# will-rowe/groot

Measured on AMD Instinct MI355X. Metric: Mreads/s aligned, higher is better.
Workload: dtype u64

## Files before the change

groot_amd/csrc/hip/align.hip:

```cpp
#include <hip/hip_runtime.h>

#include "kernels_align.hpp"
#include "kernels_lean.hpp"
#include "launch.hpp"

namespace groot {

void launch_align(uint32_t pw, const AlignArgs &a, dim3 grid, hipStream_t st)
{
    const size_t lds = a.lds_stride_dw ? (size_t)kBlock * a.lds_stride_dw * 4 + 16 : 0;
    if (pw == 3) {
        if (lds) hipLaunchKernelGGL((align_kernel<3, true>), grid, dim3(kBlock), lds, st, a);
        else hipLaunchKernelGGL((align_kernel<3, false>), grid, dim3(kBlock), 0, st, a);
    } else if (pw == 11) {
        if (lds) hipLaunchKernelGGL((align_kernel<11, true>), grid, dim3(kBlock), lds, st, a);
        else hipLaunchKernelGGL((align_kernel<11, false>), grid, dim3(kBlock), 0, st, a);
    }
}

void launch_align_lean(uint32_t pw, const LeanArgs &a, dim3 grid, hipStream_t st)
{
    if (pw != 3) return;
    const size_t lds = (size_t)kBlock * a.lds_stride_dw * 4;
    if (a.max_len <= 128) hipLaunchKernelGGL((align_lean_kernel<3, 4>), grid, dim3(kBlock), lds, st, a);
    else if (a.max_len <= 160) hipLaunchKernelGGL((align_lean_kernel<3, 5>), grid, dim3(kBlock), lds, st, a);
    else hipLaunchKernelGGL((align_lean_kernel<3, 8>), grid, dim3(kBlock), lds, st, a);
}

}
```

groot_amd/csrc/hip/device_types.hpp:

```cpp
#pragma once

#include <cstdint>

#include <hip/hip_runtime.h>

#include "groot_hip.h"

namespace groot {

constexpr int kBlock = 256;
constexpr uint32_t kEmpty = 0xFFFFFFFFu;

enum : uint32_t {
    kFlagShortRead = 1u,
    kFlagLongRead = 2u,
    kFlagSeedOverflow = 4u,
    kFlagTravOverflow = 8u,
    kFlagOrdOverflow = 16u,
    kFlagOvfOverflow = 32u,
    kFlagQOverflow = 64u,
};

constexpr uint32_t kIncrCap = 8;
constexpr uint32_t kIncrCapBig = 2048;
constexpr uint32_t kSeedShards = 64, kSeedShardStride = 16;
constexpr uint32_t kOvfShards = 256;

struct DeviceCounters {
    unsigned long long mapped, multimapped, alignments, seeds, revcomp_panics, short_reads;
    unsigned int n_trav;
    unsigned int max_seeds;
    unsigned int flags;
    unsigned int q_rows;
    unsigned int mask_words;
    unsigned int todo_reads;
    unsigned int seeded_reads;
    unsigned int tab_reads;
    unsigned int lean_reads;
    unsigned long long dbg[192];
};

template <int PW> struct alignas(16) NodeRec {
    uint32_t seq_off;
    uint32_t seq_len;
    uint32_t deg;
    uint8_t child_first[4];
    uint64_t first8;
    uint32_t edges[4];
    uint64_t mask[PW];
};
static_assert(sizeof(NodeRec<3>) == 64, "node record must be one 64-byte line");
static_assert(sizeof(NodeRec<11>) == 128, "wide node record must be 128 bytes");

struct alignas(16) WinRec {
    uint32_t graph;
    uint32_t node;
    uint32_t offset;
    uint32_t l1_hi;
    uint32_t cn_off, cn_end;
    uint32_t seed_s0, seed_len;
};
static_assert(sizeof(WinRec) == 32, "window record is two 16-byte words");

struct alignas(16) ReadRec {
    uint64_t seq_off;
    uint32_t len;
    uint32_t cnt_flags;
    uint32_t seed[4];
};
static_assert(sizeof(ReadRec) == 32, "read record is two 16-byte words");

constexpr uint32_t kRecCountMask = 0x00FFFFFFu;
constexpr uint32_t kRecNo12F = 1u << 24, kRecNo3F = 1u << 25, kRecNo4F = 1u << 26;
constexpr uint32_t kRecPacked = 1u << 31;
constexpr uint32_t kRecAscending = 1u << 30;
constexpr uint32_t kLongListCap = 1u << 20, kSortSeedsMax = 512;
constexpr uint32_t kSplitMin = 8, kSplitMaxItems = 256;
constexpr uint32_t kRecSplit = 1u << 23;
constexpr uint32_t kPrefixWords = 256;

struct groot_ctrav {
    uint32_t node, offset;
    uint32_t read_flags;
};
static_assert(sizeof(groot_ctrav) == 12, "packed traversal record is 12 bytes");

constexpr uint32_t kOutHdrDw = 6, kOutSeedDw = 4;
constexpr uint32_t kOutTab = 0x80000000u;
constexpr uint32_t kOutMaxTrav = 4095, kOutIdxBits = 25, kOutTravShift = 27, kOutTravLong = 15;
constexpr uint32_t kOutNoRec = 1u << 25;
constexpr uint32_t kOutAllSeeds = 1u << 26;
constexpr uint32_t kTabSeedsHere = 0x40000000u;
constexpr uint32_t kTabCounted = 0x80000000u;
__host__ __device__ inline uint32_t out_stride_q(uint32_t pw)
{
    uint32_t q = 4;
    while (q * 16 < (kOutHdrDw + kOutSeedDw) * 4 + 8 * pw) q <<= 1;
    return q;
}

__host__ __device__ constexpr uint32_t text_key_dwords(uint32_t dw) { return dw <= 7 ? 7u : dw <= 8 ? 8u : 14u; }
__host__ __device__ constexpr uint32_t text_exc_dwords(uint32_t tw)
{
    return tw > 14 ? 0u : ((2 + tw) % 4 ? 4 - (2 + tw) % 4 : (tw <= 10 ? 4u : 0u));
}

struct ExactEntry { uint32_t tag; uint32_t id; };

struct alignas(32) SigEntry {
    uint32_t id;
    uint32_t cls;
    uint32_t text_len;
    uint32_t group;
    uint8_t verdict[2][8];
};
static_assert(sizeof(SigEntry) == 32, "signature entry is two 16-byte words");
constexpr uint32_t kSigInline = 1u << 30;
constexpr uint32_t kTextMax = 256;
__host__ __device__ inline uint32_t sig_text_pack(uint32_t len, uint32_t argmin_fwd, uint32_t argmin_rc) { return len | (argmin_fwd << 10) | (argmin_rc << 20); }
__host__ __device__ inline uint32_t sig_text_len(uint32_t v) { return v & 1023u; }
__host__ __device__ inline uint32_t sig_text_argmin(uint32_t v, uint32_t row) { return (v >> (10 + 10 * row)) & 1023u; }
// ... 70 lines not shown
struct AlignArgs {
    DeviceIndex ix;
    const uint8_t *seq;
    const uint64_t *seq_off;
    uint32_t n_reads, first_read_id;
    uint32_t seed_slots;
    const uint32_t *seed_count;
    const uint32_t *seed_win;
    const uint32_t *perm;
    const ReadRec *read_rec;
    uint32_t no_align, update_weights;
    const void *node_rec;
    uint32_t *attempts;
    groot_trav *trav_first;
    uint64_t *mask_first;
    uint32_t *trav_cnt;
    groot_trav *ovf_trav;
    uint64_t *ovf_mask;
    uint32_t *ovf_cnt;
    uint32_t ovf_cap;
    uint64_t *stk_hdr;
    uint64_t *stk_mask;
    uint32_t n_threads, stk_depth;
    uint32_t lds_stride_dw;
    uint32_t *incr_cnt, *incr_win;
    uint32_t incr_cap;
    uint32_t head_lanes;
    uint32_t round_lanes;
    const uint4 *vitem;
    const uint32_t *vcount;
    uint32_t vcap;
    const uint32_t *n_perm;
    uint32_t refill;
    DeviceCounters *ctr;
};

struct alignas(16) LeanNode {
    uint32_t seq_off;
    uint32_t seq_len;
    uint32_t deg_kids;
    uint32_t pad;
    uint32_t edges[4];
    uint64_t first32;
    uint64_t mask[3];
};
static_assert(sizeof(LeanNode) == 64, "lean node record is one 64-byte line");
constexpr uint32_t kLeanNo = 0x80000000u;
struct alignas(16) LeanExt {
    uint64_t b[7];
    uint64_t pad;
};
static_assert(sizeof(LeanExt) == 64, "lean node extension is one 64-byte line");
constexpr uint32_t kLeanMaxLen = 256;

struct LeanArgs {
    const LeanNode *nodes;
    const LeanExt *ext;
    const uint32_t *bases2;
    const uint4 *cn_pre2;
    const uint64_t *node_l2b;
    const uint8_t *win_ok;
    const WinRec *win_rec;
    const uint32_t *q_row;
    const uint8_t *seq;
    const uint4 *packed;
    uint32_t packed_q;
    const uint32_t *perm;
    const ReadRec *read_rec;
    uint32_t n_reads, first_read_id, n_windows, k;
    uint32_t update_weights;
    uint32_t lds_stride_dw;
    uint32_t max_len;
    uint32_t *attempts;
    groot_trav *trav_first;
    uint64_t *mask_first;
    uint32_t *trav_cnt;
    uint8_t *defer;
    uint4 *stk;
    groot_trav *ovf_trav;
    uint64_t *ovf_mask;
    uint32_t *ovf_cnt;
    uint32_t ovf_cap;
    DeviceCounters *ctr;
};

__host__ __device__ inline uint32_t lean_stride_dw(uint32_t max_len) { return (((max_len + 15u) >> 4) + 15u) | 1u; }

}
```

groot_amd/csrc/hip/groot_hip.hip:

```cpp
#include <cstring>

#include <hip/hip_runtime.h>
#include <rocprim/rocprim.hpp>

#include <dlfcn.h>

#include <algorithm>
#include <cmath>
#include <cstdarg>
#include <cstdio>
#include <atomic>
#include <chrono>
#include <deque>
#include <memory>
#include <numeric>
#include <string>
#include <thread>
#include <vector>

#include "../common/cpus.hpp"
#include "../common/view_check.hpp"
#include "kernels_misc.hpp"
#include "launch.hpp"

using namespace groot;

template <class T> struct DevBuf {
    T *p = nullptr;
    size_t n = 0;
    hipError_t alloc(size_t count)
    {
        release();
        n = count;
        return hipMalloc((void **)&p, std::max<size_t>(count, 1) * sizeof(T));
    }
    hipError_t reserve(size_t count) { return count <= n && p ? hipSuccess : alloc(count); }
    void release()
    {
        if (p) (void)hipFree(p);
        p = nullptr;
        n = 0;
    }
    ~DevBuf() { release(); }
};

template <class T> struct PinBuf {
    T *p = nullptr;
    size_t n = 0;
    hipError_t alloc(size_t count)
    {
        release();
        n = count;
        return hipHostMalloc((void **)&p, std::max<size_t>(count, 1) * sizeof(T), hipHostMallocDefault);
    }
    hipError_t reserve(size_t count) { return count <= n && p ? hipSuccess : alloc(count); }
    void release()
    {
        if (p) (void)hipHostFree(p);
        p = nullptr;
        n = 0;
    }
    ~PinBuf() { release(); }
};

struct Knobs {
    bool no_outcome_table = false, no_text_table = false, no_sig = false, force_rccl = false, small_buffers = false, open_stats = false, poison = false, lean = false;
    static Knobs read()
    {
        Knobs k;
        k.no_outcome_table = getenv("GROOT_NO_OUTCOME_TABLE") != nullptr; k.no_text_table = getenv("GROOT_NO_TEXT_TABLE") != nullptr;
        k.no_sig = getenv("GROOT_NO_SIG") != nullptr;                     k.force_rccl = getenv("GROOT_FORCE_RCCL") != nullptr;
        k.small_buffers = getenv("GROOT_TEST_SMALL_BUFFERS") != nullptr;  k.open_stats = getenv("GROOT_OPEN_STATS") != nullptr;
        k.poison = getenv("GROOT_TEST_POISON") != nullptr;
        k.lean = getenv("GROOT_LEAN") != nullptr;
        return k;
    }
};

struct Slot {
    enum State { FREE, ACQUIRED, IN_FLIGHT, D2H_ISSUED, COLLECTED };
    State state = FREE;
    uint64_t ticket = 0;
    uint32_t n_reads = 0, first_read_id = 0, max_len = 0;
    uint32_t set = 0;
    uint32_t uniform_len = 0;
    bool mixed_len = false;
    bool text_used = false;
    bool sig_used = false;
    uint32_t packed_q = 0;
    bool lean_used = false;
    bool one_len = false;
    uint64_t n_bases = 0, n_exc = 0;
    enum Input { IN_ASCII, IN_PACKED, IN_PACKED16, IN_DEVICE } input = IN_ASCII;
    const uint8_t *ext_seq = nullptr;
    const uint64_t *ext_off = nullptr;
    PinBuf<uint8_t> h_bases;
    PinBuf<uint16_t> h_len;
    PinBuf<uint64_t> h_off, h_exc_pos;
    PinBuf<uint8_t> h_exc_byte;
    DevBuf<uint16_t> d_len;
    DevBuf<uint32_t> d_packed;
    bool exc_at_home = false;
    DevBuf<uint8_t> d_seq, d_exc_byte;
    DevBuf<uint64_t> d_off, d_exc_pos;
    uint32_t trav_cap = 0;
    DevBuf<groot_trav> d_trav;
    DevBuf<uint64_t> d_mask;
    DevBuf<DeviceCounters> d_ctr;
    PinBuf<DeviceCounters> h_ctr;
    PinBuf<groot_trav> h_trav;
    DevBuf<groot_ctrav> d_ctrav;
    PinBuf<groot_ctrav> h_ctrav;
    PinBuf<uint8_t> h_mask;
    PinBuf<uint32_t> h_ckpt;
    DevBuf<uint8_t> d_cmask;
    DevBuf<uint32_t> d_mwords, d_moff, d_ckpt;
    uint32_t n_trav = 0, copied = 0;
    uint64_t n_mask_bytes = 0, copied_bytes = 0;
    bool host_results = false;
    hipEvent_t ev_seed = nullptr;
    hipEvent_t ev_h2d0 = nullptr, ev_h2d = nullptr, ev_compute = nullptr, ev_ctr = nullptr, ev_d2h0 = nullptr, ev_d2h = nullptr;
    hipEvent_t ev[14]{};
    groot_counts counts{};
    int status = GROOT_OK;
    std::string status_msg;
    groot_stage_ms ms{};
    const uint8_t *seq() const { return input == IN_DEVICE ? ext_seq : d_seq.p; }
    const uint64_t *off() const { return input == IN_DEVICE ? ext_off : d_off.p; }
};

struct WorkSet {
    DevBuf<uint32_t> seed_count, seed_win, perm, perm_count, trav_cnt, tab_idx;
    DevBuf<uint32_t> perm2, perm2_count;
    DevBuf<uint8_t> defer;
    DevBuf<uint4> packed;
    DevBuf<ReadRec> read_rec;
    DevBuf<uint4> vitem, split_list;
    DevBuf<uint32_t> vcount;
    DevBuf<groot_trav> trav_first;
    DevBuf<uint64_t> mask_first, sketches;
    hipEvent_t ev_free = nullptr;
    bool used = false;
    Slot *owner = nullptr;
    uint64_t ticket = 0;
};

struct groot_ctx {
    int device = 0;
    std::string err;
    groot_params prm{};
    Knobs kn;
    uint32_t s = 0, k = 0, max_k = 0, l_max = 0, pw_view = 0, pw = 0, n_windows = 0, max_q = 0, band_hash_bits = 0;
    hipEvent_t h2d_last = nullptr;
    Slot *newest = nullptr;
    hipEvent_t last_compute = nullptr;
    hipStream_t own_stream = nullptr, stream = nullptr, astream = nullptr, h2d_stream = nullptr, d2h_stream = nullptr;
    bool profiling = false;

    DevBuf<uint32_t> graph_win_end;
    DevBuf<uint4> cn_pre;
    DevBuf<uint64_t> node_l2b;
    DevBuf<uint32_t> win_prefix, edges, win_graph, cn_node,
        band_keys, band_ids;
    DevBuf<ExactEntry> band_hash;
    DevBuf<uint8_t> band_sig;
    DevBuf<uint32_t> band_run;
    DevBuf<uint8_t> bases, q_k, q_l;
    DevBuf<uint16_t> q_min_eq;
    DevBuf<uint64_t> win_sketch;
    DevBuf<unsigned char> node_rec;
    DevBuf<LeanExt> lean_ext;
    DevBuf<LeanNode> lean_nodes;
    DevBuf<uint32_t> bases2;
    DevBuf<uint4> cn_pre2;
    DevBuf<uint8_t> win_ok;
    DevBuf<uint4> lean_stk;
    bool lean = false;
    DevBuf<WinRec> win_rec;
    DevBuf<ExactEntry> exact;
    DevBuf<SigEntry> sig;
    DevBuf<uint4> sig_dir;
    DevBuf<uint8_t> win_text, win_nodes;
    DevBuf<uint32_t> sig_info;
    DevBuf<uint4> out_tab;
    std::vector<uint32_t> h_out_tab;
    uint64_t out_strings = 0, out_tabulated = 0, out_entries = 0;
    double out_build_ms = 0, open_ms = 0;
    uint32_t incr_cap = kIncrCap;
    bool tab_capture = false;
    DevBuf<uint32_t> tab_idx, tab_hist, incr_cnt, incr_win;
    DevBuf<uint4> text_tab;
    uint64_t text_entries = 0;
    uint32_t batches_without_text = 0, text_retry_gap = 8;
    double text_hit_frac = 1.0;
    std::vector<uint16_t> h_q_min_eq;
    uint32_t sig_disabled = 0;
    DeviceIndex dix{};

    std::thread bg;
    std::atomic<int> bg_state{0};
    std::atomic<bool> bg_cancel{false};
    int bg_rc = 0;
    std::string bg_err;
    DeviceIndex bg_dix{};
    uint32_t bg_seed_slots = 0, bg_max_read_len = 0;
    hipStream_t bg_stream = nullptr;
    DevBuf<unsigned long long> bg_shards;
    DeviceIndex *build_dix = nullptr;
    hipStream_t build_stream = nullptr;
    unsigned long long *build_shards = nullptr;

    std::vector<std::unique_ptr<Slot>> slots;
    std::deque<Slot *> inflight;
    uint64_t next_ticket = 1;
    Slot *waited = nullptr;
    double todo_frac = 1.0;
    double lean_left_frac = 1.0;
    uint32_t n_cu = 256;
    double dfs_frac = 1.0;
    double trav_per_read = 1.25;
    double bytes_per_trav = 0;
    bool packed_travs = false;
    std::vector<uint32_t> h_node_graph;
    DevBuf<uint8_t> graph_words;
    std::vector<uint8_t> h_graph_words;
    WorkSet ws[2];
    uint32_t next_set = 0;

    uint32_t seed_slots = 0;
    DevBuf<uint32_t> sort_key, sort_key_out, perm_in, todo_list, todo_count;
    DevBuf<uint32_t> long_list, long_count;
    uint32_t vcap = 0;
    uint32_t lsh_defer_rows = 0, lsh_cap = 0;
    DevBuf<unsigned long long> seed_shards;
    DevBuf<uint32_t> lsh_list, lsh_count;
    DevBuf<uint64_t> lsh_sketch;
    DevBuf<char> sort_tmp, in_tmp;
    uint32_t ovf_cap = 0;
    DevBuf<groot_trav> ovf_trav;
    DevBuf<uint64_t> ovf_mask;
    DevBuf<uint32_t> trav_off, ovf_cnt;
    DevBuf<char> scan_tmp;
    uint32_t align_threads = 0, stk_depth = 0;
    DevBuf<uint64_t> stk_hdr, stk_mask;
    DevBuf<uint32_t> attempts, q_row, q_seen, q_of_row, q_nrows;
    uint32_t *attempts_ptr = nullptr;
    uint32_t att_cap = 0;
    bool att_external = false;
};

__attribute__((constructor)) static void groot_hw_queues() { setenv("GPU_MAX_HW_QUEUES", "8", 0); }

static thread_local std::string g_open_err;

static thread_local bool tl_background = false;

static int fail(groot_ctx *ctx, int code, const char *fmt, ...)
{
    char buf[1024];
    va_list ap;
    va_start(ap, fmt);
    vsnprintf(buf, sizeof buf, fmt, ap);
    va_end(ap);
    if (ctx) (tl_background ? ctx->bg_err : ctx->err) = buf;
    else g_open_err = buf;
    return code;
}

#define HIP_TRY(ctx, expr)                                                                             \
    do {                                                                                                \
        hipError_t e__ = (expr);                                                                        \
        if (e__ != hipSuccess) return fail(ctx, GROOT_E_DEVICE, "%s: %s", #expr, hipGetErrorString(e__)); \
    } while (0)

template <class T> static hipError_t upload(DevBuf<T> &d, const T *src, size_t n, size_t pad = 0)
{
    hipError_t e = d.alloc(n + pad);
    if (e != hipSuccess) return e;
    if (pad) {
        e = hipMemset(d.p, 0, (n + pad) * sizeof(T));
        if (e != hipSuccess) return e;
    }
    if (n) e = hipMemcpy(d.p, src, n * sizeof(T), hipMemcpyHostToDevice);
    return e;
}

namespace {

struct KLProb {
    int x, q, l, k;
    double p(double t) const { return 1.0 - std::pow(1.0 - std::pow(t / (1.0 + double(x) / double(q) - t), double(k)), double(l)); }
};

template <class F> double integrate(F f, double a, double b, double precision)
{
    double area = 0.0;
    for (double x = a; x < b; x += precision) area += f(x + 0.5 * precision) * precision;
    return area;
}

void optimal_kl(int max_k, int max_l, int x, int q, double t, int &opt_k, int &opt_l)
{
    const double prec = 0.01;
    double min_err = 1.7976931348623157e308;
    opt_k = 0; opt_l = 0;
    const double xq = double(x) / double(q);
    for (int l = 1; l <= max_l; l++)
        for (int k = 1; k <= max_k; k++) {
            KLProb pr{x, q, l, k};
            double fp = 0.0, fn = 0.0;
            if (xq >= 1.0) {
                fp = integrate([&](double v) { return pr.p(v); }, 0.0, t, prec);
                fn = integrate([&](double v) { return 1.0 - pr.p(v); }, t, 1.0, prec);
            } else if (xq >= t) {
                fp = integrate([&](double v) { return pr.p(v); }, 0.0, t, prec);
                fn = integrate([&](double v) { return 1.0 - pr.p(v); }, t, xq, prec);
            }
            const double err = fn + fp;
            if (min_err > err) { min_err = err; opt_k = k; opt_l = l; }
        }
}

uint32_t min_equal_slots(uint32_t s, int q_size, int x_size, double t)
{
    if (q_size == 0 || x_size == 0) return s + 1;
    for (uint32_t eq = 1; eq <= s; eq++) {
        const double jaccard = double(eq) / double(s);
        const double c = (double(x_size) / double(q_size) + 1.0) * jaccard / (1.0 + jaccard);
        if (c > t) return eq;
    }
    return s + 1;
}

uint32_t round_pw(uint32_t pw)
{
    for (uint32_t c : {3u, 11u})
        if (pw <= c) return c;
    return 0;
}

template <int PW> void build_node_records(const groot_index_view *v, std::vector<unsigned char> &out)
{
    std::vector<NodeRec<PW>> recs(v->n_nodes);
    for (uint32_t n = 0; n < v->n_nodes; n++) {
        NodeRec<PW> &r = recs[n];
        memset(&r, 0, sizeof r);
        r.seq_off = v->node_seq_off[n];
        r.seq_len = v->node_seq_off[n + 1] - v->node_seq_off[n];
        const uint32_t e0 = v->node_edge_off[n], deg = v->node_edge_off[n + 1] - e0;
        bool wild = false;
        for (uint32_t i = 0; i < r.seq_len; i++) wild |= v->bases[r.seq_off + i] == 'N';
        r.deg = deg | (wild ? 0x80000000u : 0u);
        if (deg <= 4) {
            for (uint32_t e = 0; e < deg; e++) {
                const uint32_t c = v->edges[e0 + e];
                r.edges[e] = c;
                r.child_first[e] = v->node_seq_off[c] < v->node_seq_off[c + 1] ? v->bases[v->node_seq_off[c]] : (uint8_t)0;
            }
        } else {
            r.edges[0] = e0;
        }
        for (uint32_t i = 0; i < 8 && i < r.seq_len; i++) r.first8 |= (uint64_t)v->bases[r.seq_off + i] << (8 * i);
        for (uint32_t w = 0; w < v->path_words; w++) r.mask[w] = v->node_mask[(size_t)n * v->path_words + w];
    }
    out.resize(recs.size() * sizeof(NodeRec<PW>));
    if (!recs.empty()) memcpy(out.data(), recs.data(), out.size());
}

}

static constexpr uint32_t kMaxLdsReadBytes = 64 * 1024;

static int alloc_seed_slots(groot_ctx *c, uint32_t slots)
{
    c->seed_slots = slots;
    for (WorkSet &w : c->ws) { HIP_TRY(c, w.seed_win.alloc((size_t)slots * c->prm.max_batch_reads)); w.owner = nullptr; w.ticket = 0; }
    return GROOT_OK;
}

static int alloc_trav(groot_ctx *c, Slot *s, uint32_t cap)
{
    s->trav_cap = cap;
    HIP_TRY(c, s->d_trav.alloc((size_t)cap + 2));
    HIP_TRY(c, s->d_mask.alloc((size_t)cap * c->pw_view + 2));
    if (!c->prm.results_on_device) {
        HIP_TRY(c, s->h_trav.alloc((size_t)cap + 2));
        HIP_TRY(c, s->h_mask.alloc((size_t)cap * c->pw_view * 8 + 16));
        HIP_TRY(c, s->h_ckpt.alloc((size_t)cap / 256 + 2));
        HIP_TRY(c, s->d_cmask.alloc((size_t)cap * c->pw_view * 8 + 16));
        HIP_TRY(c, s->d_mwords.alloc(cap));
        HIP_TRY(c, s->d_moff.alloc(cap));
        HIP_TRY(c, s->d_ckpt.alloc((size_t)cap / 256 + 2));
        if (c->packed_travs) {
            HIP_TRY(c, s->d_ctrav.alloc((size_t)cap + 2));
            HIP_TRY(c, s->h_ctrav.alloc((size_t)cap + 2));
        }
    }
    return GROOT_OK;
}

static int alloc_ovf(groot_ctx *c, uint32_t cap_per_shard)
{
    c->ovf_cap = cap_per_shard;
    HIP_TRY(c, c->ovf_trav.alloc((size_t)kOvfShards * cap_per_shard));
    HIP_TRY(c, c->ovf_mask.alloc((size_t)kOvfShards * cap_per_shard * c->pw));
    return GROOT_OK;
}

static int grow_attempts(groot_ctx *c, uint32_t rows)
{
    if (c->att_external) return fail(c, GROOT_E_NOSPACE, "a kmerCount outside the fixed layout of groot_hip_attempts_layout occurred");
    DevBuf<uint32_t> bigger;
    HIP_TRY(c, bigger.alloc((size_t)rows * c->n_windows));
    HIP_TRY(c, hipMemset(bigger.p, 0, (size_t)rows * c->n_windows * sizeof(uint32_t)));
    if (c->attempts.p && c->att_cap)
        HIP_TRY(c, hipMemcpy(bigger.p, c->attempts.p, (size_t)std::min(rows, c->att_cap) * c->n_windows * sizeof(uint32_t), hipMemcpyDeviceToDevice));
    std::swap(c->attempts.p, bigger.p);
    std::swap(c->attempts.n, bigger.n);
    c->attempts_ptr = c->attempts.p;
    c->att_cap = rows;
    return GROOT_OK;
// ... 15 lines not shown
#define GROOT_HEAVY_BLOCKS 16384u
#endif
#ifndef GROOT_SORTLIST_BLOCKS
#define GROOT_SORTLIST_BLOCKS 16384
#endif
static int launch_seed_stage(groot_ctx *c, Slot *s, bool update_weights)
{
    WorkSet *w = &c->ws[s->set];
    SeedArgs a{};
    s->packed_q = 0;
    a.ix = c->dix;
    a.seq = s->seq();
    a.seq_off = s->off();
    a.n_reads = s->n_reads;
    a.max_read_len = c->prm.max_read_len;
    const uint64_t want = (uint64_t)kBlock * s->max_len + 32;
    a.lds_read_bytes = (uint32_t)std::min<uint64_t>(want, kMaxLdsReadBytes);
    a.seed_slots = c->seed_slots;
    a.seed_count = w->seed_count.p;
    a.seed_win = w->seed_win.p;
    a.sketch_out = c->prm.keep_sketches ? w->sketches.p : nullptr;
    a.sort_key = c->sort_key.p;
    a.read_rec = w->read_rec.p;
    a.q_seen = c->q_seen.p;
    a.trav_cnt = w->trav_cnt.p;
    a.shards = c->seed_shards.p;
    a.ctr = s->d_ctr.p;
    a.long_list = c->long_list.p; a.long_count = c->long_count.p;
    if (c->dix.out_tab) {
        a.tab_idx = w->tab_idx.p;
        a.tab_hist = c->tab_hist.p;
    }
    unsigned win_bits = 2;
    for (uint32_t v = c->n_windows ? c->n_windows - 1 : 0; v; v >>= 1) win_bits++;
    win_bits = std::min(32u, std::max(3u, win_bits));
    a.sort_span_bits = std::min((unsigned)GROOT_SPAN_BITS, 32u - win_bits);
    if (win_bits - 2u + a.sort_span_bits > 24u && win_bits - 2u + 4u <= 24u) a.sort_span_bits = 24u - (win_bits - 2u);
    a.sort_span_shift = win_bits;
    const unsigned begin_bit = 2u, end_bit = win_bits + a.sort_span_bits;
    const dim3 grid((s->n_reads + kBlock - 1) / kBlock);
#ifndef GROOT_LIST_BLOCKS_MIN
#define GROOT_LIST_BLOCKS_MIN 1280
#endif
    const uint32_t list_blocks = std::max<uint32_t>(GROOT_LIST_BLOCKS_MIN, (uint32_t)std::min<double>(4.0e6, c->todo_frac * 1.25 * (double)s->n_reads / kBlock + 1.0));
    bool sig_useful = true;
    if (s->one_len && s->max_len >= c->k) {
        const uint32_t q = s->max_len - c->k + 1;
        sig_useful = q < c->h_q_min_eq.size() && c->h_q_min_eq[q] == c->s;
    }
    s->sig_used = c->dix.sig && !c->prm.keep_sketches && sig_useful;
    const double list_below = kSparseBelow;
    const bool list_mode = c->dfs_frac < list_below;
    const bool text_try = c->text_hit_frac >= 0.7 || ++c->batches_without_text >= c->text_retry_gap;
    s->text_used = !c->prm.keep_sketches && c->dix.text_tab && c->dix.out_tab && text_try && s->max_len >= c->dix.w && !c->tab_capture;
    if (s->text_used) c->batches_without_text = 0;
    if (c->lsh_list.p && !c->prm.keep_sketches) {
        a.lsh_list = c->lsh_list.p; a.lsh_count = c->lsh_count.p; a.lsh_sketch = c->lsh_sketch.p;
        a.lsh_defer_rows = c->lsh_defer_rows; a.lsh_cap = c->lsh_cap;
        HIP_TRY(c, hipMemsetAsync(c->lsh_count.p, 0, 2 * sizeof(uint32_t), c->stream));
    }
    HIP_TRY(c, hipMemsetAsync(w->vcount.p, 0, 2 * sizeof(uint32_t), c->stream));
    if (c->profiling) HIP_TRY(c, hipEventRecord(s->ev[7], c->stream));
    if (s->text_used) {
        a.todo_list = c->todo_list.p;
        a.todo_count = c->todo_count.p;
        const uint32_t stride_dw = ((s->max_len + 3) / 4 + 1) | 1u;
        a.list_stride_dw = list_lds_stride(stride_dw);
        const size_t lds = kTextBad + (size_t)((a.lds_read_bytes + 15) / 16) * 4 + 96;
        HIP_TRY(c, hipMemsetAsync(c->todo_count.p, 0, sizeof(uint32_t), c->stream));
        if (list_mode) {
            a.dfs_list = w->perm.p; a.dfs_count = w->perm_count.p;
            HIP_TRY(c, hipMemsetAsync(w->perm_count.p, 0, sizeof(uint32_t), c->stream));
        }
        launch_text_lookup(text_key_dwords((c->dix.w + 15) / 16), a, grid, lds, c->stream);
        HIP_TRY(c, hipGetLastError());
        if (c->profiling) HIP_TRY(c, hipEventRecord(s->ev[8], c->stream));
        launch_list(c->s, a, dim3(std::min<uint32_t>(grid.x, list_blocks)), c->stream);
    } else if (s->sig_used) {
        a.todo_list = c->todo_list.p;
        a.todo_count = c->todo_count.p;
        const uint32_t stride_dw = ((s->max_len + 3) / 4 + 1) | 1u;
        a.list_stride_dw = list_lds_stride(stride_dw);
        HIP_TRY(c, hipMemsetAsync(c->todo_count.p, 0, sizeof(uint32_t), c->stream));
        if (c->lean && !c->tab_capture && w->packed.p) { a.packed = w->packed.p; a.packed_q = s->max_len <= 128 ? 2u : 4u; }
        s->packed_q = a.packed ? a.packed_q : 0;
        launch_sig(c->s, a, s->max_len, c->stream);
        HIP_TRY(c, hipGetLastError());
        if (c->profiling) HIP_TRY(c, hipEventRecord(s->ev[8], c->stream));
        launch_list(c->s, a, dim3(std::min<uint32_t>(grid.x, list_blocks)), c->stream);
    } else {
        const size_t lds = kLdsReads + ((a.lds_read_bytes + 15) & ~15u);
        launch_seed(c->s, c->max_k, a, c->prm.keep_sketches != 0, grid, lds, c->stream);
        HIP_TRY(c, hipGetLastError());
        if (c->profiling) HIP_TRY(c, hipEventRecord(s->ev[8], c->stream));
    }
    if (a.lsh_list) hipLaunchKernelGGL(lsh_heavy_kernel, dim3(std::min<uint32_t>(grid.x, GROOT_HEAVY_BLOCKS)), dim3(kBlock), 0, c->stream, a);
    HIP_TRY(c, hipGetLastError());
    if (c->profiling) HIP_TRY(c, hipEventRecord(s->ev[12], c->stream));
    {
        SplitArgs sa{};
        sa.list = c->long_list.p; sa.count = c->long_count.p; sa.seed_count = w->seed_count.p; sa.seed_win = w->seed_win.p;
        sa.n_reads = s->n_reads; sa.seed_slots = c->seed_slots; sa.read_rec = w->read_rec.p; sa.win_rec = c->dix.win_rec;
        sa.split = c->vcap && !c->tab_capture && !c->prm.no_exact_align;
        sa.vitem = w->vitem.p; sa.vcount = w->vcount.p; sa.vcap = c->vcap; sa.split_list = w->split_list.p;
        sa.ctr = s->d_ctr.p; sa.update_weights = update_weights ? 1 : 0;
        hipLaunchKernelGGL(sort_seed_lists_kernel, dim3(GROOT_SORTLIST_BLOCKS), dim3(kBlock), 0, c->stream, sa);
    }
    if (c->profiling) HIP_TRY(c, hipEventRecord(s->ev[2], c->stream));
    hipLaunchKernelGGL(assign_q_rows_kernel, dim3(1), dim3(64), 0, c->stream, c->q_seen.p, c->q_row.p, c->q_of_row.p, c->q_nrows.p, c->att_cap,
                       c->max_q, s->d_ctr.p, c->seed_shards.p, c->long_count.p);
    if (a.tab_hist) {
        hipLaunchKernelGGL(fold_tab_hist_kernel, dim3(std::min<uint32_t>((c->n_windows + kBlock - 1) / kBlock, 1024u)), dim3(kBlock), 0, c->stream, c->tab_hist.p,
                           c->attempts_ptr, c->q_row.p, c->dix.w - c->k + 1, c->n_windows, s->d_ctr.p, update_weights ? 1u : 0u);
        HIP_TRY(c, hipGetLastError());
    }
    if (list_mode && a.dfs_list) return GROOT_OK;
    if (list_mode) {
        size_t tb = 0;
        HasKey pred{c->sort_key.p};
        rocprim::counting_iterator<uint32_t> ids(0u);
        HIP_TRY(c, rocprim::select(nullptr, tb, ids, w->perm.p, w->perm_count.p, (size_t)s->n_reads, pred, c->stream));
        if (tb > c->sort_tmp.n) {
            HIP_TRY(c, hipStreamSynchronize(c->stream));
            HIP_TRY(c, c->sort_tmp.alloc(tb + tb / 4));
        }
        HIP_TRY(c, rocprim::select(c->sort_tmp.p, tb, ids, w->perm.p, w->perm_count.p, (size_t)s->n_reads, pred, c->stream));
        return GROOT_OK;
    }
    size_t tmp_bytes = 0;
    HIP_TRY(c, rocprim::radix_sort_pairs(nullptr, tmp_bytes, c->sort_key.p, c->sort_key_out.p, c->perm_in.p, w->perm.p, s->n_reads, begin_bit,
                                         end_bit, c->stream));
    if (tmp_bytes > c->sort_tmp.n) {
        HIP_TRY(c, hipStreamSynchronize(c->stream));
        HIP_TRY(c, c->sort_tmp.alloc(tmp_bytes + tmp_bytes / 4));
    }
    HIP_TRY(c, rocprim::radix_sort_pairs(c->sort_tmp.p, tmp_bytes, c->sort_key.p, c->sort_key_out.p, c->perm_in.p, w->perm.p,
                                         s->n_reads, begin_bit, end_bit, c->stream));
    return GROOT_OK;
}

struct LeanLeft {
    const uint8_t *defer;
    const DeviceCounters *ctr;
    uint32_t lean_slots;
    __device__ uint8_t operator()(uint32_t i) const { return i < ctr->seeded_reads && (i >= lean_slots || defer[i]) ? 1 : 0; }
};

static int launch_align_stage(groot_ctx *c, Slot *s, bool update_weights)
{
    WorkSet *w = &c->ws[s->set];
    AlignArgs a{};
    a.ix = c->dix;
    a.seq = s->seq();
    a.seq_off = s->off();
    a.n_reads = s->n_reads;
    a.first_read_id = s->first_read_id;
    a.seed_slots = c->seed_slots;
    a.seed_count = w->seed_count.p;
    a.seed_win = w->seed_win.p;
    a.perm = w->perm.p;
    a.read_rec = w->read_rec.p;
    a.no_align = c->prm.no_exact_align;
    a.update_weights = update_weights ? 1 : 0;
    a.attempts = c->attempts_ptr;
    a.node_rec = c->node_rec.p;
    a.trav_first = w->trav_first.p;
    a.mask_first = w->mask_first.p;
    a.trav_cnt = w->trav_cnt.p;
    a.ovf_trav = c->ovf_trav.p;
    a.ovf_mask = c->ovf_mask.p;
    a.ovf_cnt = c->ovf_cnt.p;
    a.ovf_cap = c->ovf_cap;
    if (c->vcap) { a.vitem = w->vitem.p; a.vcount = w->vcount.p; a.vcap = c->vcap; }
    a.stk_hdr = c->stk_hdr.p;
    a.stk_mask = c->stk_mask.p;
    uint32_t blocks = std::min<uint32_t>((s->n_reads + kBlock - 1) / kBlock, c->align_threads / kBlock);
    if (c->dfs_frac < kSparseBelow && c->dfs_frac * (double)s->n_reads < 16.0 * (double)(blocks * (kBlock / 64))) blocks = std::max(1u, blocks / 2);
    else if (c->dfs_frac >= kSparseBelow && c->dfs_frac < 0.6 && !s->mixed_len && blocks >= 4) blocks /= 2;
    if (c->lean && !c->tab_capture && c->lean_left_frac < 0.25) {
        uint32_t want = (uint32_t)(c->lean_left_frac * 1.25 * (double)s->n_reads / 64.0 / (kBlock / 64)) + 1u;
        blocks = std::max(1u, std::min(blocks, std::max(want, c->n_cu)));
    }
    a.n_threads = blocks * kBlock;
    a.stk_depth = c->stk_depth;
    {
        const uint32_t stride = (2 + 4 * ((s->max_len + 27) / 16)) | 1u;
        a.lds_stride_dw = (size_t)kBlock * stride * 4 <= 64 * 1024 ? stride : 0;
    }
    if (c->tab_capture) {
        a.incr_cnt = c->incr_cnt.p; a.incr_win = c->incr_win.p; a.incr_cap = c->incr_cap;
        HIP_TRY(c, hipMemsetAsync(c->incr_cnt.p, 0, (size_t)s->n_reads * sizeof(uint32_t), c->astream));
    }
    a.head_lanes = s->mixed_len ? 16u : 0u;
#ifndef GROOT_REFILL_ERR
#define GROOT_REFILL_ERR 48
#endif
#ifndef GROOT_REFILL_MIXED
#define GROOT_REFILL_MIXED 2
#endif
    a.refill = s->mixed_len ? (uint32_t)GROOT_REFILL_MIXED : (c->dfs_frac >= kSparseBelow && c->dfs_frac < 0.6 ? (uint32_t)GROOT_REFILL_ERR : 64u);
#ifdef GROOT_WORK_COUNTERS
    if (const char *e = getenv("GROOT_DEV_ROUND")) a.round_lanes = (uint32_t)atoi(e);
#endif
    a.ctr = s->d_ctr.p;
    HIP_TRY(c, hipMemsetAsync(c->ovf_cnt.p, 0, (kOvfShards + 2) * sizeof(uint32_t), c->astream));
    const uint32_t lean_stride = lean_stride_dw(s->max_len);
    s->lean_used = c->lean && !c->tab_capture && s->n_reads && s->max_len <= kLeanMaxLen && c->dfs_frac >= 0.02;
    if (s->lean_used) {
        LeanArgs l{};
        l.nodes = c->lean_nodes.p; l.ext = c->lean_ext.p; l.bases2 = c->bases2.p; l.cn_pre2 = c->cn_pre2.p; l.win_ok = c->win_ok.p;
        l.win_rec = c->dix.win_rec; l.node_l2b = c->dix.node_l2b; l.q_row = c->q_row.p;
        l.seq = s->seq(); l.packed = s->packed_q ? w->packed.p : nullptr; l.packed_q = s->packed_q; l.perm = w->perm.p; l.read_rec = w->read_rec.p;
        l.n_reads = s->n_reads; l.first_read_id = s->first_read_id; l.n_windows = c->n_windows; l.k = c->k;
        l.update_weights = update_weights ? 1 : 0;
        l.lds_stride_dw = lean_stride; l.max_len = s->max_len;
        l.attempts = c->attempts_ptr;
        l.trav_first = w->trav_first.p; l.mask_first = w->mask_first.p; l.trav_cnt = w->trav_cnt.p;
        l.defer = w->defer.p; l.ctr = s->d_ctr.p;
        l.stk = c->lean_stk.p; l.ovf_trav = c->ovf_trav.p; l.ovf_mask = c->ovf_mask.p; l.ovf_cnt = c->ovf_cnt.p; l.ovf_cap = c->ovf_cap;
        const uint32_t lean_blocks = std::min<uint32_t>((s->n_reads + kBlock - 1) / kBlock, (uint32_t)(c->dfs_frac * 1.05 * (double)s->n_reads / kBlock) + 64u);
        launch_align_lean(c->pw, l, dim3(lean_blocks), c->astream);
        HIP_TRY(c, hipGetLastError());
        size_t tb = 0;
        rocprim::counting_iterator<uint32_t> ids(0u);
        auto flags = rocprim::make_transform_iterator(ids, LeanLeft{w->defer.p, s->d_ctr.p, lean_blocks * (uint32_t)kBlock});
        HIP_TRY(c, rocprim::select(nullptr, tb, w->perm.p, flags, w->perm2.p, w->perm2_count.p, (size_t)s->n_reads, c->astream));
        if (tb > c->scan_tmp.n) {
            HIP_TRY(c, hipStreamSynchronize(c->astream));
            HIP_TRY(c, c->scan_tmp.alloc(tb + tb / 4));
        }
        HIP_TRY(c, rocprim::select(c->scan_tmp.p, tb, w->perm.p, flags, w->perm2.p, w->perm2_count.p, (size_t)s->n_reads, c->astream));
        a.perm = w->perm2.p;
        a.n_perm = w->perm2_count.p;
        if (c->profiling) HIP_TRY(c, hipEventRecord(s->ev[13], c->astream));
    }
    launch_align(c->pw, a, dim3(blocks), c->astream);
    HIP_TRY(c, hipGetLastError());
    return GROOT_OK;
}

static int launch_order_stage(groot_ctx *c, Slot *s, bool update_weights)
{
    WorkSet *w = &c->ws[s->set];
    const uint32_t n = s->n_reads;
    size_t tmp_bytes = 0;
    if (c->vcap) hipLaunchKernelGGL(split_fix_kernel, dim3(256), dim3(kBlock), 0, c->astream, w->split_list.p, w->vcount.p, w->vitem.p, w->trav_cnt.p, n, s->d_ctr.p,
                                    w->trav_first.p, w->mask_first.p, c->pw, s->first_read_id);
    HIP_TRY(c, rocprim::exclusive_scan(nullptr, tmp_bytes, w->trav_cnt.p, c->trav_off.p, 0u, n, rocprim::plus<uint32_t>(), c->astream));
    if (tmp_bytes > c->scan_tmp.n) {
        HIP_TRY(c, hipStreamSynchronize(c->astream));
        HIP_TRY(c, c->scan_tmp.alloc(tmp_bytes + tmp_bytes / 4));
    }
    HIP_TRY(c, rocprim::exclusive_scan(c->scan_tmp.p, tmp_bytes, w->trav_cnt.p, c->trav_off.p, 0u, n, rocprim::plus<uint32_t>(), c->astream));
    hipLaunchKernelGGL(order_total_kernel, dim3(1), dim3(1), 0, c->astream, c->trav_off.p, w->trav_cnt.p, n, s->d_ctr.p);
    OrderTabArgs ot{};
    if (c->dix.out_tab) {
        ot.tab_idx = w->tab_idx.p; ot.out_tab = c->dix.out_tab; ot.stride_q = c->dix.out_stride_q; ot.first_read_id = s->first_read_id;
        ot.update_weights = update_weights ? 1 : 0;
        ot.attempts = c->attempts_ptr; ot.q_row = c->q_row.p;
        ot.q_tab = c->dix.w - c->k + 1; ot.n_windows = c->n_windows;
    }
    if (c->profiling) HIP_TRY(c, hipEventRecord(s->ev[9], c->astream));
    hipLaunchKernelGGL(order_first_kernel, dim3(std::min<uint32_t>((n + kBlock - 1) / kBlock, 2048u)), dim3(kBlock), 0, c->astream, w->trav_first.p,
                       w->mask_first.p, c->trav_off.p, w->trav_cnt.p, n, s->d_trav.p, s->d_mask.p, s->trav_cap, c->pw,
                       c->pw_view, s->d_ctr.p, ot);
    if (c->profiling) HIP_TRY(c, hipEventRecord(s->ev[10], c->astream));
    if (c->vcap) hipLaunchKernelGGL(order_split_kernel, dim3(std::min<uint32_t>((c->vcap + kBlock - 1) / kBlock, 256u)), dim3(kBlock), 0, c->astream, w->vitem.p, w->vcount.p, c->vcap, w->trav_cnt.p,
                                    c->trav_off.p, w->trav_first.p, w->mask_first.p, n, s->first_read_id, s->d_trav.p, s->d_mask.p, s->trav_cap, c->pw, c->pw_view, s->d_ctr.p);
    hipLaunchKernelGGL(order_ovf_kernel, dim3((c->ovf_cap + kBlock - 1) / kBlock, kOvfShards), dim3(kBlock), 0, c->astream,
                       c->ovf_trav.p, c->ovf_mask.p, c->ovf_cnt.p, c->ovf_cap, c->trav_off.p, s->first_read_id, s->d_trav.p,
                       s->d_mask.p, s->trav_cap, c->pw, c->pw_view, s->d_ctr.p, w->vitem.p, n);
    HIP_TRY(c, hipGetLastError());
    if (!c->prm.results_on_device) {
        const dim3 g((s->trav_cap + kBlock - 1) / kBlock);
        hipLaunchKernelGGL(mask_words_kernel, g, dim3(kBlock), 0, c->astream, s->d_trav.p, s->d_ctr.p, s->trav_cap, c->graph_words.p, (uint32_t)c->h_graph_words.size(),
                           s->d_mwords.p);
        size_t tb = 0;
        HIP_TRY(c, rocprim::exclusive_scan(nullptr, tb, s->d_mwords.p, s->d_moff.p, 0u, s->trav_cap, rocprim::plus<uint32_t>(), c->astream));
        if (tb > c->scan_tmp.n) {
            HIP_TRY(c, hipStreamSynchronize(c->astream));
            HIP_TRY(c, c->scan_tmp.alloc(tb + tb / 4));
        }
        HIP_TRY(c, rocprim::exclusive_scan(c->scan_tmp.p, tb, s->d_mwords.p, s->d_moff.p, 0u, s->trav_cap, rocprim::plus<uint32_t>(), c->astream));
        hipLaunchKernelGGL(mask_compact_kernel, g, dim3(kBlock), 0, c->astream, s->d_trav.p, s->d_mask.p, c->pw_view, s->d_ctr.p, s->trav_cap,
                           c->graph_words.p, (uint32_t)c->h_graph_words.size(), s->d_moff.p, s->d_cmask.p, s->d_ckpt.p);
        if (c->packed_travs) hipLaunchKernelGGL(trav_pack_kernel, g, dim3(kBlock), 0, c->astream, s->d_trav.p, s->d_ctr.p, s->trav_cap, s->first_read_id, s->d_ctrav.p);
        HIP_TRY(c, hipGetLastError());
    }
    return GROOT_OK;
}

static int run_batch_async(groot_ctx *c, Slot *s, bool update_weights)
{
    WorkSet *w = &c->ws[s->set];
    if (w->used) HIP_TRY(c, hipStreamWaitEvent(c->stream, w->ev_free, 0));
    HIP_TRY(c, hipMemsetAsync(s->d_ctr.p, 0, sizeof(DeviceCounters), c->stream));
    if (c->kn.poison) {
        const size_t n = s->n_reads;
        HIP_TRY(c, hipMemsetAsync(w->seed_count.p, 0, n * sizeof(uint32_t), c->stream));
        HIP_TRY(c, hipMemsetAsync(w->read_rec.p, 0, n * sizeof(ReadRec), c->stream));
        HIP_TRY(c, hipMemsetAsync(w->trav_cnt.p, 0, n * sizeof(uint32_t), c->stream));
        HIP_TRY(c, hipMemsetAsync(c->sort_key.p, 0xFF, n * sizeof(uint32_t), c->stream));
        if (w->tab_idx.p) HIP_TRY(c, hipMemsetAsync(w->tab_idx.p, 0xFF, n * sizeof(uint32_t), c->stream));
        HIP_TRY(c, hipMemsetAsync(c->todo_list.p, 0, n * sizeof(uint32_t), c->stream));
// ... 180 lines not shown
static void expand_travs(const groot_ctx *c, Slot *s)
{
    const size_t n = s->n_trav;
    const groot_ctrav *in = s->h_ctrav.p;
    groot_trav *out = s->h_trav.p;
    const uint32_t first = s->first_read_id;
    const uint32_t *node_graph = c->h_node_graph.data();
    auto span = [=](size_t lo, size_t hi) {
        if (lo >= hi) return;
        uint32_t ord = 0, prev = ~0u;
        if (lo) {
            prev = in[lo - 1].read_flags & 0x00FFFFFFu;
            if ((in[lo].read_flags & 0x00FFFFFFu) == prev) {
                size_t j = lo;
                while (j > 0 && (in[j - 1].read_flags & 0x00FFFFFFu) == prev) j--;
                ord = (uint32_t)(lo - j) - 1;
            }
        }
        for (size_t i = lo; i < hi; i++) {
            const uint32_t pos = in[i].read_flags & 0x00FFFFFFu;
            ord = pos == prev ? ord + 1 : 0;
            prev = pos;
            groot_trav t;
            t.read_id = first + pos; t.graph_id = node_graph[in[i].node]; t.node = in[i].node; t.offset = in[i].offset;
            t.ord = (uint16_t)ord; t.flags = (uint8_t)(in[i].read_flags >> 24); t.reserved = 0;
            out[i] = t;
        }
    };
    const unsigned nt = (unsigned)std::min<size_t>(std::min(16u, granted_cpus()), n / (1u << 18));
    if (nt <= 1) { span(0, n); return; }
    std::vector<std::thread> th;
    const size_t per = (n + nt - 1) / nt;
    for (unsigned t = 0; t < nt; t++) th.emplace_back(span, std::min(n, t * per), std::min(n, (t + 1) * per));
    for (auto &x : th) x.join();
}

static int finish_counters(groot_ctx *c, Slot *s)
{
    DeviceCounters &h = *s->h_ctr.p;
    auto refetch = [&](DeviceCounters &dst) -> int {
        HIP_TRY(c, hipMemcpyAsync(s->h_ctr.p, s->d_ctr.p, sizeof(DeviceCounters), hipMemcpyDeviceToHost, c->astream));
        HIP_TRY(c, hipStreamSynchronize(c->astream));
        dst = *s->h_ctr.p;
        return GROOT_OK;
    };
    DeviceCounters first = h;
    bool have_first = false;
    bool redone = false;
    for (int attempt = 0; s->n_reads; attempt++) {
        const uint32_t fl = h.flags;
        if (!(fl & (kFlagSeedOverflow | kFlagQOverflow | kFlagOvfOverflow | kFlagTravOverflow))) break;
        if (attempt > 8) return fail(c, GROOT_E_NOSPACE, "output buffers keep overflowing (flags=0x%x)", fl);
        HIP_TRY(c, hipStreamSynchronize(c->stream));
        HIP_TRY(c, hipStreamSynchronize(c->astream));
        bool redo_weights = !have_first;
        if (fl & (kFlagSeedOverflow | kFlagQOverflow)) {
            if (fl & kFlagSeedOverflow) { if (int rc = alloc_seed_slots(c, h.max_seeds + 4)) return rc; }
            if (fl & kFlagQOverflow) {
                if (c->att_external) {
                    s->status = GROOT_E_NOSPACE;
                    s->status_msg = "a kmerCount outside the fixed layout of groot_hip_attempts_layout occurred";
                    h.n_trav = 0;
                    break;
                }
                if (int rc = grow_attempts(c, std::max(h.q_rows, c->att_cap * 2))) return rc;
            }
        } else {
            if (!have_first) { first = h; have_first = true; }
            redo_weights = false;
            if (fl & kFlagOvfOverflow) { if (int rc = alloc_ovf(c, c->ovf_cap * 4)) return rc; }
            if (fl & kFlagTravOverflow) { if (int rc = alloc_trav(c, s, h.n_trav + h.n_trav / 8 + 1024)) return rc; }
        }
        if (int rc = run_batch_async(c, s, redo_weights)) return rc;
        redone = true;
        DeviceCounters again{};
        if (int rc = refetch(again)) return rc;
        if (have_first) {
            const uint32_t keep = first.flags & ~(kFlagOvfOverflow | kFlagTravOverflow | kFlagSeedOverflow | kFlagQOverflow);
            DeviceCounters merged = first;
            merged.n_trav = again.n_trav; merged.alignments = again.alignments; merged.seeds = again.seeds; merged.max_seeds = again.max_seeds;
            merged.flags = keep | again.flags;
            merged.q_rows = again.q_rows;
            merged.mask_words = again.mask_words;
            merged.todo_reads = again.todo_reads; merged.tab_reads = again.tab_reads; merged.lean_reads = again.lean_reads;
            h = merged;
        } else h = again;
    }
    s->n_trav = s->n_reads ? h.n_trav : 0;
    groot_counts &o = s->counts;
    o.received = s->n_reads;
    o.mapped = h.mapped; o.multimapped = h.multimapped; o.alignments = h.alignments; o.seeds = h.seeds;
    o.travs = s->n_trav; o.revcomp_panics = h.revcomp_panics; o.short_reads = h.short_reads;
    o.full_sketch_reads = (s->sig_used || s->text_used) ? h.todo_reads : s->n_reads;
    o.walked_reads = h.seeded_reads;
    o.lean_reads = h.lean_reads;
    if (s->status == GROOT_OK) {
        char buf[256];
        if (h.flags & kFlagLongRead) { s->status = GROOT_E_NOSPACE; snprintf(buf, sizeof buf, "a read is longer than max_read_len=%u", c->prm.max_read_len); s->status_msg = buf; }
        else if (h.flags & kFlagOrdOverflow) { s->status = GROOT_E_NOSPACE; s->status_msg = "a read produced more than 65535 traversals"; }
        else if (h.flags & kFlagShortRead) {
            s->status = GROOT_E_SHORT_READ;
            snprintf(buf, sizeof buf, "k size is greater than sequence length for %llu read(s) (the reference panics: boss.go:164-166)", h.short_reads);
            s->status_msg = buf;
        } else if (h.revcomp_panics) {
            s->status = GROOT_E_REVCOMP;
            snprintf(buf, sizeof buf, "%llu read(s) hold a byte > 'T' and reached RevComplement (the reference panics: seqio.go:126)", h.revcomp_panics);
            s->status_msg = buf;
        }
    }
#if defined(GROOT_WORK_COUNTERS) && GROOT_WORK_COUNTERS == 3
    if (h.dbg[4]) {
        fprintf(stderr, "[groot timeline] wavefronts with work %llu, rounds %llu, iterations: mean %.0f max %llu; wave duration: mean %.3f ms max %.3f ms\n", h.dbg[4], h.dbg[5],
                (double)h.dbg[0] / (double)h.dbg[4], h.dbg[1], (double)h.dbg[2] / (double)h.dbg[4] / 1e5, (double)h.dbg[3] / 1e5);
        for (unsigned long long i = 0; i < 14 && i < h.dbg[17]; i++)
            fprintf(stderr, "[groot timeline] late read %llu%s: %llu windows, %llu graphs, %llu traversals, from %llu to %llu us, %llu wave iterations, %llu steps of its own\n", h.dbg[18 + 3 * i] & 0xFFFFFFFFull,
                    (h.dbg[18 + 3 * i] >> 63) ? " (item)" : "", (h.dbg[18 + 3 * i] >> 32) & 0x7FFFFFFFull, h.dbg[20 + 3 * i] >> 56, (h.dbg[20 + 3 * i] >> 48) & 0xFFull, h.dbg[19 + 3 * i] & 0xFFFFFFFFull, h.dbg[19 + 3 * i] >> 32,
                    h.dbg[20 + 3 * i] & 0xFFFFFFFFull, (h.dbg[20 + 3 * i] >> 32) & 0xFFFFull);
        fprintf(stderr, "[groot timeline] late reads in all: %llu\n", h.dbg[17]);
        fprintf(stderr, "[groot timeline] ms summed over wavefronts: all %.1f = cooperative scans %.1f (%llu services) + fork/join %.1f + FETCH %.1f (%llu steps) + SCAN %.1f (%llu) + DFS %.1f (%llu) + rest\n",
                (double)h.dbg[2] / 1e5, (double)h.dbg[8] / 1e5, h.dbg[16], (double)h.dbg[9] / 1e5, (double)h.dbg[10] / 1e5, h.dbg[13], (double)h.dbg[11] / 1e5, h.dbg[14], (double)h.dbg[12] / 1e5, h.dbg[15]);
        for (int hh = 0; hh < 2; hh++) {
            fprintf(stderr, "[groot timeline] %s (buckets of 50 us):", hh ? "length of a wavefront's last round" : "wavefront ends after");
            for (int b = 0; b < 64; b++) fprintf(stderr, " %llu", h.dbg[64 + 64 * hh + b]);
            fprintf(stderr, "\n");
        }
    }
#elif defined(GROOT_WORK_COUNTERS) && GROOT_WORK_COUNTERS == 4
    if (h.dbg[151]) {
        const double nw = (double)h.dbg[151];
        fprintf(stderr, "[groot lean] wavefronts %llu; per wavefront: %.1f iterations (with a level-1 / level-2 / level-3-4 / walk lane: %.1f / %.1f / %.1f / %.1f); lane-steps per wavefront: %.0f / %.0f / %.0f / %.0f; staging %.2f us, loop %.2f us\n",
                h.dbg[151], (double)h.dbg[148] / nw, (double)h.dbg[140] / nw, (double)h.dbg[141] / nw, (double)h.dbg[142] / nw, (double)h.dbg[143] / nw,
                (double)h.dbg[144] / nw, (double)h.dbg[145] / nw, (double)h.dbg[146] / nw, (double)h.dbg[147] / nw, (double)h.dbg[149] / nw / 100.0, (double)h.dbg[150] / nw / 100.0);
        fprintf(stderr, "[groot lean] finished without an alignment %llu; left to align_kernel: seeds > 4: %llu, byte > T / length: %llu, byte other than ACGT: %llu, window with an N: %llu, node with an N: %llu, N ahead: %llu, three neighbours: %llu, third pending: %llu, too many steps: %llu\n",
                h.dbg[160], h.dbg[161], h.dbg[163], h.dbg[164], h.dbg[165], h.dbg[166], h.dbg[167], h.dbg[168], h.dbg[169], h.dbg[170]);
    }
#elif defined(GROOT_WORK_COUNTERS)
    for (int e = 0; e < 32; e++)
        if (h.dbg[e]) fprintf(stderr, "[groot work] event %2d: wave iterations %llu lanes %llu\n", e, h.dbg[e], h.dbg[32 + e]);
    fprintf(stderr, "[groot work] longest round: %llu wave iterations\n", h.dbg[63]);
#if GROOT_WORK_COUNTERS == 2
    fprintf(stderr, "[groot work] slow reads (%llu):", h.dbg[128]);
    for (int i = 0; i < 30 && (unsigned long long)i < h.dbg[128]; i++)
        fprintf(stderr, " %llu:%llu:%llu/%llu/%llu", h.dbg[129 + 2 * i] & 0xFFFFFFFFull, h.dbg[129 + 2 * i] >> 32, h.dbg[130 + 2 * i] & 0xFFFFFull,
                (h.dbg[130 + 2 * i] >> 20) & 0xFFFFFull, h.dbg[130 + 2 * i] >> 40);
    fprintf(stderr, "\n");
#endif
    for (int i = 0; i < 5; i++) fprintf(stderr, "[groot work] FETCH part %d: %.1f ms summed over wavefronts\n", i, (double)h.dbg[40 + i] / 1e5);
    for (int ph = 0; ph < 3; ph++)
        fprintf(stderr, "[groot work] phase %d: %llu steps, %.2f us per step (wall clock, per wave)\n", ph, h.dbg[27 + ph],
                h.dbg[27 + ph] ? (double)h.dbg[24 + ph] / 100.0 / (double)h.dbg[27 + ph] : 0.0);
    for (int hh = 0; hh < 2; hh++) {
        fprintf(stderr, "[groot work] %s (buckets of 2 iterations):", hh ? "round length" : "lane finish");
        for (int b = 0; b < 64; b++) fprintf(stderr, " %llu", h.dbg[64 + 64 * hh + b]);
        fprintf(stderr, "\n");
    }
#endif
    if (s->n_reads) c->trav_per_read = (double)s->n_trav / (double)s->n_reads;
    if (s->n_reads && !c->tab_capture) c->dfs_frac = (double)h.seeded_reads / (double)s->n_reads;
    if (s->n_reads && !c->tab_capture && s->lean_used) c->lean_left_frac = (double)(h.seeded_reads - std::min(h.seeded_reads, h.lean_reads)) / (double)s->n_reads;
    if (s->n_reads && (s->sig_used || s->text_used)) c->todo_frac = (double)h.todo_reads / (double)s->n_reads;
    if (s->n_reads && !c->tab_capture && c->dix.text_tab) {
        c->text_hit_frac = s->text_used ? 1.0 - (double)h.todo_reads / (double)s->n_reads : (double)h.tab_reads / (double)s->n_reads;
        if (s->text_used) c->text_retry_gap = c->text_hit_frac >= 0.7 ? 8u : std::min(256u, c->text_retry_gap * 2u);
    }
    s->n_mask_bytes = s->n_trav ? h.mask_words : 0;
    if (!c->prm.results_on_device && s->n_trav) {
        c->bytes_per_trav = (double)s->n_mask_bytes / (double)s->n_trav;
        const uint32_t have = redone ? 0 : std::min(s->copied, s->n_trav);
        if (have < s->n_trav) {
            if (c->packed_travs) HIP_TRY(c, hipMemcpy(s->h_ctrav.p + have, s->d_ctrav.p + have, (size_t)(s->n_trav - have) * sizeof(groot_ctrav), hipMemcpyDeviceToHost));
            else HIP_TRY(c, hipMemcpy(s->h_trav.p + have, s->d_trav.p + have, (size_t)(s->n_trav - have) * sizeof(groot_trav), hipMemcpyDeviceToHost));
            HIP_TRY(c, hipMemcpy(s->h_ckpt.p, s->d_ckpt.p, ((size_t)s->n_trav / 256 + 1) * sizeof(uint32_t), hipMemcpyDeviceToHost));
        }
        const uint64_t have_w = redone ? 0 : std::min<uint64_t>(s->copied_bytes, s->n_mask_bytes);
        if (have_w < s->n_mask_bytes)
            HIP_TRY(c, hipMemcpy(s->h_mask.p + have_w, s->d_cmask.p + have_w, (size_t)(s->n_mask_bytes - have_w), hipMemcpyDeviceToHost));
        if (c->packed_travs) expand_travs(c, s);
        s->host_results = true;
    }
    s->state = Slot::D2H_ISSUED;
    return GROOT_OK;
}

static int progress(groot_ctx *c, Slot *must = nullptr)
{
    bool blocking = must != nullptr;
    for (Slot *s : c->inflight) {
        if (s->state == Slot::IN_FLIGHT) {
            if (blocking) HIP_TRY(c, hipEventSynchronize(s->ev_ctr));
            else {
                const hipError_t q = hipEventQuery(s->ev_ctr);
                if (q == hipErrorNotReady) break;
                if (q != hipSuccess) return fail(c, GROOT_E_DEVICE, "hipEventQuery: %s", hipGetErrorString(q));
            }
            if (int rc = finish_counters(c, s)) return rc;
        }
        if (s == must) blocking = false;
    }
    return GROOT_OK;
}

static int collect_impl(groot_ctx *c, Slot **out)
{
    if (c->inflight.empty()) return fail(c, GROOT_E_STATE, "no batch submitted");
    HIP_TRY(c, hipSetDevice(c->device));
    Slot *s = c->inflight.front();
    if (s->state == Slot::IN_FLIGHT) {
        if (int rc = progress(c, s)) return rc;
    }
    if (c->profiling && s->n_reads) {
        if (s->input != Slot::IN_DEVICE) (void)hipEventElapsedTime(&s->ms.h2d, s->ev_h2d0, s->ev_h2d);
        (void)hipEventElapsedTime(&s->ms.unpack, s->ev[0], s->ev[1]);
        (void)hipEventElapsedTime(&s->ms.sketch_seed, s->ev[1], s->ev[2]);
        (void)hipEventElapsedTime(&s->ms.schedule, s->ev[2], s->ev[3]);
        (void)hipEventElapsedTime(&s->ms.align, s->ev[11], s->ev[4]);
        (void)hipEventElapsedTime(&s->ms.sort, s->ev[4], s->ev[5]);
        (void)hipEventElapsedTime(&s->ms.total, s->ev[0], s->ev[5]);
        (void)hipEventElapsedTime(&s->ms.first_seed_kernel, s->ev[7], s->ev[8]);
        (void)hipEventElapsedTime(&s->ms.order_kernel, s->ev[9], s->ev[10]);
        (void)hipEventElapsedTime(&s->ms.list_pass, s->ev[8], s->ev[12]);
        s->ms.lean_pass = 0;
        if (s->lean_used) (void)hipEventElapsedTime(&s->ms.lean_pass, s->ev[11], s->ev[13]);
        (void)hipEventElapsedTime(&s->ms.wall, s->ev[1], s->ev[5]);
        if (!c->prm.results_on_device) (void)hipEventElapsedTime(&s->ms.d2h, s->ev_d2h0, s->ev_d2h);
    }
    c->inflight.pop_front();
    s->state = Slot::COLLECTED;
    *out = s;
    (void)progress(c);
    return GROOT_OK;
}

static int drain(groot_ctx *c)
{
    HIP_TRY(c, hipSetDevice(c->device));
    if (!c->inflight.empty()) { if (int rc = progress(c, c->inflight.back())) return rc; }
    HIP_TRY(c, hipStreamSynchronize(c->stream));
    HIP_TRY(c, hipStreamSynchronize(c->astream));
    HIP_TRY(c, hipStreamSynchronize(c->d2h_stream));
    return GROOT_OK;
}

extern "C" {

void groot_params_default(groot_params *p)
{
    if (!p) return;
    memset(p, 0, sizeof *p);
    p->containment_threshold = 0.99;
    p->max_read_len = 256;
    p->max_batch_reads = 1u << 20;
    p->max_seeds_per_read = 8;
    p->pipeline_depth = 3;
}

int groot_hip_device_count(int *n)
{
    if (!n) return GROOT_E_INVALID;
    int c = 0;
    hipError_t e = hipGetDeviceCount(&c);
    if (e != hipSuccess) {
        *n = 0;
        return fail(nullptr, GROOT_E_DEVICE, "hipGetDeviceCount: %s", hipGetErrorString(e));
    }
    *n = c;
    return GROOT_OK;
}

const char *groot_hip_last_error(const groot_ctx *ctx) { return ctx ? ctx->err.c_str() : g_open_err.c_str(); }

void groot_hip_close(groot_ctx *ctx)
{
    if (!ctx) return;
    (void)hipSetDevice(ctx->device);
    ctx->bg_cancel = true;
    if (ctx->bg.joinable()) ctx->bg.join();
    if (ctx->bg_stream) { (void)hipStreamSynchronize(ctx->bg_stream); (void)hipStreamDestroy(ctx->bg_stream); }
    if (ctx->stream) (void)hipStreamSynchronize(ctx->stream);
    if (ctx->astream) (void)hipStreamSynchronize(ctx->astream);
    if (ctx->h2d_stream) (void)hipStreamSynchronize(ctx->h2d_stream);
    if (ctx->d2h_stream) (void)hipStreamSynchronize(ctx->d2h_stream);
    for (auto &s : ctx->slots) {
        for (hipEvent_t e : {s->ev_seed, s->ev_h2d0, s->ev_h2d, s->ev_compute, s->ev_ctr, s->ev_d2h0, s->ev_d2h})
            if (e) (void)hipEventDestroy(e);
        for (auto &e : s->ev)
            if (e) (void)hipEventDestroy(e);
    }
    ctx->slots.clear();
    for (WorkSet &w : ctx->ws)
        if (w.ev_free) (void)hipEventDestroy(w.ev_free);
    if (ctx->own_stream) (void)hipStreamDestroy(ctx->own_stream);
    if (ctx->astream) (void)hipStreamDestroy(ctx->astream);
    if (ctx->h2d_stream) (void)hipStreamDestroy(ctx->h2d_stream);
    if (ctx->d2h_stream) (void)hipStreamDestroy(ctx->d2h_stream);
    delete ctx;
}

static int text_pass(groot_ctx *c, const uint8_t *seqs, const uint32_t *owner, uint32_t n, uint32_t len, uint8_t *differs, uint32_t *cnt_flags,
                     uint32_t *keys)
{
    DevBuf<uint64_t> off, sk;
    DevBuf<uint8_t> seq, bad;
    DevBuf<DeviceCounters> ctr;
    DevBuf<uint32_t> cnt, win, key, own;
    DevBuf<ReadRec> rec;
// ... 608 lines not shown
    c->build_dix = &c->dix; c->build_stream = c->stream; c->build_shards = c->seed_shards.p;
    if (st == 3) return fail(c, c->bg_rc ? c->bg_rc : GROOT_E_DEVICE, "background part of groot_hip_open: %s", c->bg_err.c_str());
    if (st == 4) return GROOT_OK;
    const DeviceIndex &b = c->bg_dix;
    c->dix.win_prefix = b.win_prefix;
    c->dix.sig = b.sig; c->dix.sig_dir = b.sig_dir; c->dix.sig_mask = b.sig_mask; c->dix.win_text = b.win_text;
    c->dix.sig_info = b.sig_info; c->dix.sig_verdict_stride = b.sig_verdict_stride; c->dix.win_nodes = b.win_nodes;
    return GROOT_OK;
}

static int open_impl(groot_ctx *c, int device_id, const groot_index_view *v, const groot_params *p, uint32_t flags)
{
    int ndev = 0;
    if (hipGetDeviceCount(&ndev) != hipSuccess || ndev == 0)
        return fail(c, GROOT_E_DEVICE, "no HIP device available (libgroot_hip has no CPU fallback)");
    if (device_id < 0 || device_id >= ndev) return fail(c, GROOT_E_INVALID, "device %d out of range (%d devices)", device_id, ndev);
    if (!v) return fail(c, GROOT_E_INVALID, "null index view");
    c->device = device_id;
    c->kn = Knobs::read();
    HIP_TRY(c, hipSetDevice(device_id));
    groot_params d;
    groot_params_default(&d);
    c->prm = p ? *p : d;
    if (!c->prm.max_read_len) c->prm.max_read_len = d.max_read_len;
    if (!c->prm.max_batch_reads) c->prm.max_batch_reads = d.max_batch_reads;
    if (!c->prm.max_seeds_per_read) c->prm.max_seeds_per_read = d.max_seeds_per_read;
    if (!c->prm.max_batch_bases) c->prm.max_batch_bases = (uint64_t)c->prm.max_batch_reads * c->prm.max_read_len;
    if (!c->prm.pipeline_depth) c->prm.pipeline_depth = d.pipeline_depth;
    if (c->prm.pipeline_depth > 16) return fail(c, GROOT_E_INVALID, "pipeline_depth must be <= 16");
    if (c->prm.max_read_len > 65535) return fail(c, GROOT_E_UNSUPPORTED, "max_read_len must be <= 65535");
    if (v->kmer_size == 0 || v->kmer_size > 64) return fail(c, GROOT_E_UNSUPPORTED, "k-mer size %u not in [1,64]", v->kmer_size);
    if (c->prm.max_read_len < v->kmer_size) return fail(c, GROOT_E_INVALID, "max_read_len smaller than the k-mer size");
    {
        const std::string why = check_index_view(v);
        if (!why.empty()) return fail(c, GROOT_E_FORMAT, "inconsistent index view: %s", why.c_str());
    }
    if (!seed_supported(v->sketch_size, v->max_k))
        return fail(c, GROOT_E_UNSUPPORTED, "sketch size %u with maxK %u is outside what the kernels handle (1 <= maxK <= sketch size <= %d)", v->sketch_size,
                    v->max_k, kGenericMaxS);
    c->s = v->sketch_size; c->k = v->kmer_size; c->max_k = v->max_k; c->l_max = v->sketch_size / v->max_k;
    c->pw_view = v->path_words; c->pw = round_pw(v->path_words);
    if (!c->pw) return fail(c, GROOT_E_UNSUPPORTED, "graphs with more than 704 paths are not supported (path_words=%u)", v->path_words);
    c->n_windows = v->n_windows;
    c->max_q = c->prm.max_read_len - c->k + 1;

    HIP_TRY(c, hipStreamCreateWithFlags(&c->own_stream, hipStreamNonBlocking));
    {
        int lo = 0, hi = 0;
        (void)hipDeviceGetStreamPriorityRange(&lo, &hi);
        if (hipStreamCreateWithPriority(&c->astream, hipStreamNonBlocking, lo) != hipSuccess)
            HIP_TRY(c, hipStreamCreateWithFlags(&c->astream, hipStreamNonBlocking));
    }
    for (WorkSet &w : c->ws) HIP_TRY(c, hipEventCreateWithFlags(&w.ev_free, hipEventDisableTiming));
    HIP_TRY(c, hipStreamCreateWithFlags(&c->h2d_stream, hipStreamNonBlocking));
    HIP_TRY(c, hipStreamCreateWithFlags(&c->d2h_stream, hipStreamNonBlocking));
    c->stream = c->own_stream;
    c->build_dix = &c->dix; c->build_stream = c->stream;
    for (uint32_t i = 0; i < c->prm.pipeline_depth; i++) {
        std::unique_ptr<Slot> s(new Slot());
        for (hipEvent_t *e : {&s->ev_seed, &s->ev_h2d0, &s->ev_h2d, &s->ev_compute, &s->ev_ctr, &s->ev_d2h0, &s->ev_d2h}) HIP_TRY(c, hipEventCreate(e));
        for (auto &e : s->ev) HIP_TRY(c, hipEventCreate(&e));
        c->slots.push_back(std::move(s));
    }

    const bool open_stats = c->kn.open_stats;
    auto t_open = std::chrono::steady_clock::now();
    auto lap = [&](const char *what) {
        if (!open_stats) return;
        (void)hipDeviceSynchronize();
        const auto now = std::chrono::steady_clock::now();
        fprintf(stderr, "[groot open] %-28s %8.1f ms\n", what, std::chrono::duration<double, std::milli>(now - t_open).count());
        t_open = now;
    };
    lap("device + streams");
    HIP_TRY(c, upload(c->edges, v->edges, v->n_edges));
    HIP_TRY(c, upload(c->bases, v->bases, v->n_bases, 64));
    {
        std::vector<unsigned char> recs;
        if (c->pw == 3) build_node_records<3>(v, recs);
        else build_node_records<11>(v, recs);
        HIP_TRY(c, upload(c->node_rec, recs.data(), recs.size()));
    }
    c->lean = c->pw == 3 && c->kn.lean && !c->prm.no_exact_align;
    if (c->lean) {
        auto code_of = [](uint8_t b) -> int { return b == 'A' ? 0 : b == 'C' ? 1 : b == 'T' ? 2 : b == 'G' ? 3 : -1; };
        std::vector<uint32_t> b2((size_t)(v->n_bases + 15) / 16 + 20, 0);
        for (uint64_t i = 0; i < v->n_bases; i++) {
            const int cd = code_of(v->bases[i]);
            if (cd > 0) b2[i >> 4] |= (uint32_t)cd << (2 * (i & 15));
        }
        std::vector<LeanNode> ln(v->n_nodes);
        std::vector<LeanExt> lx(v->n_nodes);
        std::vector<uint8_t> node_bad(v->n_nodes, 0);
        for (uint32_t n = 0; n < v->n_nodes; n++) {
            LeanNode &r = ln[n];
            memset(&r, 0, sizeof r);
            memset(&lx[n], 0, sizeof(LeanExt));
            r.seq_off = v->node_seq_off[n];
            r.seq_len = v->node_seq_off[n + 1] - v->node_seq_off[n];
            const uint32_t e0 = v->node_edge_off[n], deg = v->node_edge_off[n + 1] - e0;
            bool no = deg > 4;
            for (uint32_t i = 0; i < r.seq_len; i++) {
                const int cd = code_of(v->bases[r.seq_off + i]);
                if (cd < 0) no = true;
                else if (i < 32) r.first32 |= (uint64_t)cd << (2 * i);
                else if (i < 256) lx[n].b[(i >> 5) - 1] |= (uint64_t)cd << (2 * (i & 31));
            }
            node_bad[n] = no;
            r.deg_kids = std::min(deg, 7u) | (no ? kLeanNo : 0u);
            for (uint32_t e = 0; e < std::min(deg, 4u); e++) {
                const uint32_t ch = v->edges[e0 + e];
                r.edges[e] = ch;
                uint32_t kid = 8;
                if (v->node_seq_off[ch] < v->node_seq_off[ch + 1]) {
                    const int cd = code_of(v->bases[v->node_seq_off[ch]]);
                    kid = cd < 0 ? 4u : (uint32_t)cd;
                }
                r.deg_kids |= kid << (8 + 4 * e);
                if (v->node_seq_off[ch + 1] - v->node_seq_off[ch] > 32u) r.deg_kids |= 1u << (24 + e);
            }
            for (uint32_t w = 0; w < v->path_words && w < 3; w++) r.mask[w] = v->node_mask[(size_t)n * v->path_words + w];
        }
        std::vector<uint32_t> pre2((size_t)v->n_cn * 4 + 4, 0);
        for (uint64_t i = 0; i < v->n_cn; i++) {
            const uint32_t nd = v->cn_node[i];
            const uint32_t s0 = v->node_seq_off[nd], nlen = v->node_seq_off[nd + 1] - s0;
            uint64_t bits = 0;
            for (uint32_t j = 0; j < std::min(nlen, 24u); j++) {
                const int cd = code_of(v->bases[s0 + j]);
                if (cd > 0) bits |= (uint64_t)cd << (2 * j);
            }
            uint32_t *e = &pre2[(size_t)i * 4];
            e[0] = (uint32_t)bits; e[1] = (uint32_t)(bits >> 32) | (std::min(nlen, 65535u) << 16); e[2] = nd; e[3] = s0;
        }
        std::vector<uint8_t> ok(v->n_windows, 1);
        for (uint32_t w = 0; w < v->n_windows; w++) {
            if (node_bad[v->win_node[w]]) ok[w] = 0;
            for (uint32_t i = v->win_cn_off[w]; i < v->win_cn_off[w + 1]; i++) {
                const uint32_t nd = v->cn_node[i];
                if (node_bad[nd] || v->node_seq_off[nd + 1] - v->node_seq_off[nd] > 65535u) ok[w] = 0;
            }
        }
        HIP_TRY(c, upload(c->bases2, b2.data(), b2.size()));
        HIP_TRY(c, upload(c->lean_nodes, ln.data(), ln.size()));
        HIP_TRY(c, upload(c->lean_ext, lx.data(), lx.size()));
        HIP_TRY(c, upload(c->cn_pre2, reinterpret_cast<const uint4 *>(pre2.data()), pre2.size() / 4));
        HIP_TRY(c, upload(c->win_ok, ok.data(), ok.size()));
    }
    {
        std::vector<uint32_t> pre((size_t)v->n_cn * 8 + 8, 0);
        for (uint64_t i = 0; i < v->n_cn; i++) {
            const uint32_t nd = v->cn_node[i];
            const uint32_t s0 = v->node_seq_off[nd], nlen = v->node_seq_off[nd + 1] - s0;
            uint32_t *e = &pre[(size_t)i * 8];
            memcpy(e, v->bases + s0, std::min(nlen, 24u));
            e[6] = nd; e[7] = nlen;
        }
        HIP_TRY(c, upload(c->cn_pre, reinterpret_cast<const uint4 *>(pre.data()), pre.size() / 4));
        c->dix.cn_pre = c->cn_pre.p;
    }
    {
        std::vector<uint64_t> sets((size_t)v->n_nodes * 11, 0);
        const unsigned nt = std::max(1u, std::min(32u, granted_cpus()));
        std::vector<std::thread> th;
        for (unsigned t = 0; t < nt; t++)
            th.emplace_back([&, t]() {
                struct Walk {
// ... 165 lines not shown
                for (uint32_t e = n; e-- > 0;) {
                    const uint32_t *ke = &keys[((size_t)b * n + e) * mk];
                    rn[e] = (e + 1 < n && std::equal(ke, ke + K, ke + mk)) ? rn[e + 1] + 1 : 1;
                }
            }
        };
        {
            std::atomic<uint32_t> next{0};
            std::vector<std::thread> th;
            const uint32_t workers = std::min<uint32_t>(lmax, std::min(16u, granted_cpus()));
            for (uint32_t t = 0; t < workers; t++)
                th.emplace_back([&]() { for (uint32_t b; (b = next.fetch_add(1)) < lmax;) band(b); });
            for (auto &x : th) x.join();
        }
        });
    }
    auto finish_lsh = [&]() -> int {
        if (lsh.job.joinable()) lsh.job.join();
        if (c->band_keys.p) return GROOT_OK;
        HIP_TRY(c, upload(c->band_keys, lsh.keys.data(), lsh.keys.size()));
        HIP_TRY(c, upload(c->band_ids, lsh.ids.data(), lsh.ids.size()));
        HIP_TRY(c, upload(c->band_hash, lsh.tab.data(), lsh.tab.size()));
        HIP_TRY(c, upload(c->band_sig, lsh.sig.data(), lsh.sig.size(), 32));
        HIP_TRY(c, upload(c->band_run, lsh.run.data(), lsh.run.size()));
        c->dix.band_keys = c->band_keys.p; c->dix.band_ids = c->band_ids.p; c->dix.band_hash = c->band_hash.p;
        c->dix.band_sig = c->band_sig.p; c->dix.band_run = c->band_run.p;
        lsh.keys = {}; lsh.ids = {}; lsh.run = {}; lsh.tab = {}; lsh.sig = {};
        return GROOT_OK;
    };
    lap("LSH forest tables");
    {
        std::vector<uint8_t> qk(c->max_q + 1, 0), ql(c->max_q + 1, 0);
        std::vector<uint16_t> qm(c->max_q + 1, (uint16_t)(s + 1));
        for (uint32_t q = 1; q <= c->max_q; q++) {
            int K, L;
            optimal_kl((int)v->max_k, (int)c->l_max, (int)v->num_window_kmers, (int)q, c->prm.containment_threshold, K, L);
            qk[q] = (uint8_t)K; ql[q] = (uint8_t)L;
            qm[q] = (uint16_t)min_equal_slots(s, (int)q, (int)v->num_window_kmers, c->prm.containment_threshold);
        }
        HIP_TRY(c, upload(c->q_k, qk.data(), qk.size()));
        HIP_TRY(c, upload(c->q_l, ql.data(), ql.size()));
        HIP_TRY(c, upload(c->q_min_eq, qm.data(), qm.size()));
        c->h_q_min_eq = qm;
    }
    {
        std::vector<uint32_t> none(c->max_q + 2, kEmpty);
        HIP_TRY(c, upload(c->q_row, none.data(), none.size()));
        HIP_TRY(c, c->q_seen.alloc(c->max_q + 2));
        HIP_TRY(c, hipMemset(c->q_seen.p, 0, (size_t)(c->max_q + 2) * 4));
        HIP_TRY(c, c->q_of_row.alloc(c->max_q + 2));
        HIP_TRY(c, c->q_nrows.alloc(1));
        HIP_TRY(c, hipMemset(c->q_nrows.p, 0, 4));
        if (int rc = grow_attempts(c, std::min<uint32_t>(4, c->max_q + 1))) return rc;
    }
    DeviceIndex &x = c->dix;
    x.k = v->kmer_size; x.s = s; x.w = v->window_size; x.num_window_kmers = v->num_window_kmers;
    x.n_windows = n; x.n_nodes = v->n_nodes; x.pw = c->pw;
    x.edges = c->edges.p; x.bases = c->bases.p;
    x.win_prefix = c->win_prefix.p; x.win_graph = c->win_graph.p; x.win_rec = c->win_rec.p; x.cn_node = c->cn_node.p;
    x.win_sketch = c->win_sketch.p; x.exact = c->exact.p; x.band_keys = c->band_keys.p; x.band_ids = c->band_ids.p;
    x.band_hash = c->band_hash.p; x.band_hash_bits = c->band_hash_bits; x.band_sig = c->band_sig.p; x.band_run = c->band_run.p;
    x.max_k = v->max_k; x.l_max = c->l_max; x.q_k = c->q_k.p; x.q_l = c->q_l.p; x.q_min_eq = c->q_min_eq.p; x.max_q = c->max_q;
    x.q_row = c->q_row.p;

    lap("per-kmerCount tables");
    const uint32_t R = c->prm.max_batch_reads;
    HIP_TRY(c, c->sort_key.alloc(R));
    HIP_TRY(c, c->sort_key_out.alloc(R));
    HIP_TRY(c, c->long_list.alloc(kLongListCap));
    HIP_TRY(c, c->long_count.alloc(4));
    HIP_TRY(c, hipMemset(c->long_count.p, 0, 4 * sizeof(uint32_t)));
    {
        std::vector<uint32_t> iota(R);
        std::iota(iota.begin(), iota.end(), 0u);
        HIP_TRY(c, upload(c->perm_in, iota.data(), iota.size()));
    }
    if (int rc = alloc_seed_slots(c, c->prm.max_seeds_per_read)) return rc;
    c->vcap = c->kn.small_buffers ? 8u : std::max<uint32_t>(4096, R / 4);
    for (WorkSet &w : c->ws) {
        HIP_TRY(c, w.seed_count.alloc(R));
        HIP_TRY(c, w.read_rec.alloc(R));
        HIP_TRY(c, w.perm.alloc(R));
        HIP_TRY(c, w.perm_count.alloc(4));
        if (c->lean) {
            HIP_TRY(c, w.perm2.alloc(R));
            HIP_TRY(c, w.perm2_count.alloc(4));
            HIP_TRY(c, w.defer.alloc(R));
            HIP_TRY(c, w.packed.alloc((size_t)R * (c->prm.max_read_len <= 128 ? 2 : 4)));
        }
        if (c->prm.keep_sketches) HIP_TRY(c, w.sketches.alloc((size_t)R * s));
        HIP_TRY(c, w.trav_first.alloc((size_t)R + c->vcap));
        HIP_TRY(c, w.mask_first.alloc(((size_t)R + c->vcap) * c->pw));
        HIP_TRY(c, w.trav_cnt.alloc((size_t)R + c->vcap));
        HIP_TRY(c, w.vitem.alloc(std::max<uint32_t>(c->vcap, 1)));
        HIP_TRY(c, w.split_list.alloc(kLongListCap));
        HIP_TRY(c, w.vcount.alloc(4));
        HIP_TRY(c, hipMemset(w.vcount.p, 0, 4 * sizeof(uint32_t)));
    }
    HIP_TRY(c, c->trav_off.alloc(R));
    if (c->lean) HIP_TRY(c, c->lean_stk.alloc((size_t)R * 4));
    HIP_TRY(c, c->ovf_cnt.alloc(kOvfShards + 2));
    if (int rc = alloc_ovf(c, c->kn.small_buffers ? 2u : std::max<uint32_t>(256, R / kOvfShards / 4))) return rc;
    int n_cu = 256;
    (void)hipDeviceGetAttribute(&n_cu, hipDeviceAttributeMultiprocessorCount, c->device);
    c->n_cu = (uint32_t)std::max(n_cu, 1);
    uint32_t per_cu = c->pw > 3 ? kAlignWavesWide : kAlignWaves;
    c->align_threads = std::min<uint32_t>(((R + kBlock - 1) / kBlock) * kBlock, (uint32_t)std::max(n_cu, 1) * per_cu * kBlock);
    c->stk_depth = c->prm.max_read_len;
    HIP_TRY(c, c->stk_hdr.alloc((size_t)c->stk_depth * c->align_threads));
    HIP_TRY(c, c->stk_mask.alloc((size_t)c->stk_depth * c->align_threads * c->pw));
    if (c->l_max <= kLshMaxBands) {
#ifndef GROOT_LSH_DEFER_ROWS
#define GROOT_LSH_DEFER_ROWS 64
#endif
        c->lsh_defer_rows = GROOT_LSH_DEFER_ROWS;
        c->lsh_cap = c->kn.small_buffers ? 4u : std::max<uint32_t>(4096, R / 4);
        HIP_TRY(c, c->lsh_list.alloc(c->lsh_cap));
        HIP_TRY(c, c->lsh_count.alloc(4));
        HIP_TRY(c, c->lsh_sketch.alloc((size_t)c->lsh_cap * s));
    }
    HIP_TRY(c, c->todo_list.alloc(R));
    HIP_TRY(c, c->todo_count.alloc(1));
    HIP_TRY(c, c->seed_shards.alloc((size_t)kSeedShards * kSeedShardStride));
    HIP_TRY(c, hipMemset(c->seed_shards.p, 0, (size_t)kSeedShards * kSeedShardStride * sizeof(unsigned long long)));
    HIP_TRY(c, hipDeviceSynchronize());
    lap("work buffers");
    c->build_shards = c->seed_shards.p;
    const uint32_t q_w = v->window_size >= v->kmer_size ? v->window_size - v->kmer_size + 1 : 0;
    const bool w_exact = q_w && q_w < c->h_q_min_eq.size() && c->h_q_min_eq[q_w] == s;
    const bool memo_wanted = !c->kn.no_outcome_table && c->prm.memo_budget_mb != GROOT_MEMO_OFF && !c->prm.no_exact_align && !c->prm.keep_sketches;
    if ((flags & GROOT_OPEN_BACKGROUND) && !memo_wanted) {
        if (int rc = finish_lsh()) return rc;
        lap("LSH forest tables (waited for)");
        c->bg_dix = c->dix;
        HIP_TRY(c, hipStreamCreateWithFlags(&c->bg_stream, hipStreamNonBlocking));
        HIP_TRY(c, c->bg_shards.alloc((size_t)kSeedShards * kSeedShardStride));
        HIP_TRY(c, hipMemset(c->bg_shards.p, 0, (size_t)kSeedShards * kSeedShardStride * sizeof(unsigned long long)));
        c->build_dix = &c->bg_dix; c->build_stream = c->bg_stream; c->build_shards = c->bg_shards.p;
        c->bg_seed_slots = c->seed_slots; c->bg_max_read_len = c->prm.max_read_len;
        c->bg_state.store(1);
        c->bg = std::thread([c, v, sc = std::move(sketch_class)]() {
            tl_background = true;
            int rc = GROOT_OK;
            try {
                if (hipSetDevice(c->device) != hipSuccess) rc = fail(c, GROOT_E_DEVICE, "hipSetDevice");
                if (!rc && !c->bg_cancel) rc = build_prefix_tables(c, v);
                if (!rc && !c->bg_cancel) rc = build_signature_index(c, v, sc);
            } catch (const std::exception &e) {
                rc = fail(c, GROOT_E_NOSPACE, "%s", e.what());
            }
            c->bg_rc = rc;
            c->bg_state.store(rc ? 3 : (c->bg_cancel ? 4 : 2), std::memory_order_release);
        });
        return GROOT_OK;
    }
    if (int rc = build_prefix_tables(c, v)) return rc;
    lap("prefix tables");
    if (!w_exact) { if (int rc = finish_lsh()) return rc; lap("LSH forest tables (waited for)"); }
    if (int rc = build_signature_index(c, v, sketch_class)) return rc;
    if (int rc = finish_lsh()) return rc;
    lap("signature index");
    return GROOT_OK;
}

int groot_hip_open_stats(const groot_ctx *c, groot_open_stats *out)
{
    if (!c || !out) return GROOT_E_INVALID;
    memset(out, 0, sizeof *out);
    out->open_ms = c->open_ms; out->memo_ms = c->out_build_ms;
    out->memo_strings = c->out_strings; out->memo_tabulated = c->out_tabulated; out->memo_entries = c->out_entries; out->text_entries = c->text_entries;
    out->memo_hbm_bytes = c->out_tab.n * sizeof(uint4) + c->text_tab.n * sizeof(uint4) + c->sig_info.n * sizeof(uint32_t);
    return GROOT_OK;
}

int groot_hip_open(groot_ctx **out, int device_id, const groot_index_view *idx, const groot_params *p)
{
    return groot_hip_open_flags(out, device_id, idx, p, 0);
}

int groot_hip_open_abandon(groot_ctx *c)
{
    if (!c) return GROOT_E_INVALID;
    if (c->bg_state.load(std::memory_order_acquire) == 1) c->bg_cancel = true;
// ... 356 lines not shown
                const uint32_t w = c->h_graph_words[s->h_trav.p[i].graph_id];
                memcpy(masks + i * c->pw_view, s->h_mask.p + o, (size_t)w);
                o += w;
            }
        }
    } else {
        if (m && out) HIP_TRY(c, hipMemcpy(out, s->d_trav.p, m * sizeof(groot_trav), hipMemcpyDeviceToHost));
        if (m && masks) HIP_TRY(c, hipMemcpy(masks, s->d_mask.p, m * c->pw_view * sizeof(uint64_t), hipMemcpyDeviceToHost));
    }
    return GROOT_OK;
}

static int work_buffers_of_waited(groot_ctx *c)
{
    Slot *s = c->waited;
    if (!s) return fail(c, GROOT_E_STATE, "no finished batch");
    if (s->n_reads && (c->ws[s->set].owner != s || c->ws[s->set].ticket != s->ticket))
        return fail(c, GROOT_E_STATE, "a newer batch has been submitted: the seeds / sketches of the waited batch are gone");
    return GROOT_OK;
}

int groot_hip_read_seeds(groot_ctx *c, groot_seed *out, uint64_t cap, uint64_t *n)
{
    if (!c || !n) return GROOT_E_INVALID;
    if (int rc = work_buffers_of_waited(c)) return rc;
    HIP_TRY(c, hipSetDevice(c->device));
    const Slot *s = c->waited;
    const uint32_t R = s->n_reads;
    std::vector<uint32_t> cnt(R), win((size_t)c->seed_slots * R);
    if (R) {
        HIP_TRY(c, hipMemcpy(cnt.data(), c->ws[s->set].seed_count.p, (size_t)R * 4, hipMemcpyDeviceToHost));
        HIP_TRY(c, hipMemcpy(win.data(), c->ws[s->set].seed_win.p, (size_t)c->seed_slots * R * 4, hipMemcpyDeviceToHost));
    }
    std::vector<uint32_t> tidx;
    if (R && c->dix.out_tab && !c->h_out_tab.empty()) {
        tidx.resize(R);
        HIP_TRY(c, hipMemcpy(tidx.data(), c->ws[s->set].tab_idx.p, (size_t)R * 4, hipMemcpyDeviceToHost));
    }
    const size_t ed = (size_t)c->dix.out_stride_q * 4;
    uint64_t total = 0;
    std::vector<uint32_t> tmp;
    for (uint32_t r = 0; r < R; r++) {
        tmp.clear();
        if (!tidx.empty() && tidx[r] != kEmpty && (tidx[r] & kTabSeedsHere)) {
            const uint32_t *e0 = &c->h_out_tab[(size_t)(tidx[r] & ((1u << kOutIdxBits) - 1u)) * ed];
            const uint32_t n_ent = std::max(e0[3] >> 16, 1u) + (e0[2] >> 20);
            for (uint32_t e = 0; e < n_ent; e++)
                for (uint32_t x = 0; x < kOutSeedDw; x++)
                    if (e0[e * ed + ed - kOutSeedDw + x] != kEmpty) tmp.push_back(e0[e * ed + ed - kOutSeedDw + x]);
        } else {
            const uint32_t m = std::min(cnt[r] & 0x7FFFFFFFu, c->seed_slots);
            for (uint32_t j = 0; j < m; j++) tmp.push_back(win[(size_t)j * R + r]);
        }
        std::sort(tmp.begin(), tmp.end());
        for (uint32_t w : tmp) {
            if (out && total < cap) out[total] = groot_seed{s->first_read_id + r, w};
            total++;
        }
    }
    *n = total;
    return GROOT_OK;
}

int groot_hip_read_sketches(groot_ctx *c, uint64_t *out, uint64_t cap_reads, uint64_t *n_reads)
{
    if (!c || !n_reads) return GROOT_E_INVALID;
    if (int rc = work_buffers_of_waited(c)) return rc;
    if (!c->prm.keep_sketches) return fail(c, GROOT_E_STATE, "ctx was opened without keep_sketches");
    HIP_TRY(c, hipSetDevice(c->device));
    *n_reads = c->waited->n_reads;
    const uint64_t m = std::min<uint64_t>(cap_reads, c->waited->n_reads);
    if (m && out) HIP_TRY(c, hipMemcpy(out, c->ws[c->waited->set].sketches.p, m * c->s * sizeof(uint64_t), hipMemcpyDeviceToHost));
    return GROOT_OK;
}

int groot_hip_stage_ms(groot_ctx *c, groot_stage_ms *out)
{
    if (!c || !out) return GROOT_E_INVALID;
    if (c->waited) *out = c->waited->ms;
    else memset(out, 0, sizeof *out);
    return GROOT_OK;
}

static int table_rows(groot_ctx *c, std::vector<uint32_t> &q_of_row)
{
    if (int rc = drain(c)) return rc;
    uint32_t n = 0;
    HIP_TRY(c, hipMemcpy(&n, c->q_nrows.p, 4, hipMemcpyDeviceToHost));
    q_of_row.resize(n);
    if (n) HIP_TRY(c, hipMemcpy(q_of_row.data(), c->q_of_row.p, (size_t)n * 4, hipMemcpyDeviceToHost));
    return GROOT_OK;
}

int groot_hip_attempts_export(groot_ctx *c, uint32_t *q_values, uint32_t *counts, uint32_t cap_rows, uint32_t *n_rows, uint32_t *n_windows)
{
    if (!c || !n_rows) return GROOT_E_INVALID;
    std::vector<uint32_t> qs;
    if (int rc = table_rows(c, qs)) return rc;
    *n_rows = (uint32_t)qs.size();
    if (n_windows) *n_windows = c->n_windows;
    std::vector<uint32_t> order(qs.size());
    std::iota(order.begin(), order.end(), 0u);
    std::sort(order.begin(), order.end(), [&](uint32_t a, uint32_t b) { return qs[a] < qs[b]; });
    for (uint32_t i = 0; i < order.size() && i < cap_rows; i++) {
        if (q_values) q_values[i] = qs[order[i]];
        if (counts && c->n_windows)
            HIP_TRY(c, hipMemcpy(counts + (size_t)i * c->n_windows, c->attempts_ptr + (size_t)order[i] * c->n_windows, (size_t)c->n_windows * 4,
                                 hipMemcpyDeviceToHost));
    }
    return GROOT_OK;
}

int groot_hip_attempts_layout(groot_ctx *c, const uint32_t *q_values, uint32_t n_q, void *d_table)
{
    if (!c || (n_q && !q_values)) return GROOT_E_INVALID;
    if (!idle(c)) return fail(c, GROOT_E_STATE, "a batch is in flight");
    for (uint32_t i = 0; i < n_q; i++) {
        if (q_values[i] > c->max_q) return fail(c, GROOT_E_INVALID, "kmerCount %u exceeds max_read_len-k+1=%u", q_values[i], c->max_q);
        if (i && q_values[i] <= q_values[i - 1]) return fail(c, GROOT_E_INVALID, "kmerCounts must be strictly ascending");
    }
    std::vector<uint32_t> qs;
    if (int rc = table_rows(c, qs)) return rc;
    std::vector<uint32_t> new_row(qs.size());
    for (size_t r = 0; r < qs.size(); r++) {
        const uint32_t *p = std::lower_bound(q_values, q_values + n_q, qs[r]);
        if (p == q_values + n_q || *p != qs[r]) return fail(c, GROOT_E_INVALID, "the layout lacks kmerCount %u, which has counts", qs[r]);
        new_row[r] = (uint32_t)(p - q_values);
    }
    const uint32_t cap = std::max<uint32_t>(n_q, 1);
    DevBuf<uint32_t> own;
    uint32_t *dst = (uint32_t *)d_table;
    if (!dst) { HIP_TRY(c, own.alloc((size_t)cap * c->n_windows)); dst = own.p; }
    DevBuf<uint32_t> stage;
    const uint32_t *src = c->attempts_ptr;
    if (dst == c->attempts_ptr && !qs.empty()) {
        HIP_TRY(c, stage.alloc(qs.size() * (size_t)c->n_windows));
        HIP_TRY(c, hipMemcpy(stage.p, c->attempts_ptr, qs.size() * (size_t)c->n_windows * 4, hipMemcpyDeviceToDevice));
        src = stage.p;
    }
    if (n_q) HIP_TRY(c, hipMemset(dst, 0, (size_t)n_q * c->n_windows * 4));
    for (size_t r = 0; r < qs.size(); r++)
        HIP_TRY(c, hipMemcpy(dst + (size_t)new_row[r] * c->n_windows, src + r * c->n_windows, (size_t)c->n_windows * 4, hipMemcpyDeviceToDevice));
    std::vector<uint32_t> rowmap(c->max_q + 2, kEmpty);
    for (uint32_t i = 0; i < n_q; i++) rowmap[q_values[i]] = i;
    HIP_TRY(c, hipMemcpy(c->q_row.p, rowmap.data(), rowmap.size() * 4, hipMemcpyHostToDevice));
    if (n_q) HIP_TRY(c, hipMemcpy(c->q_of_row.p, q_values, (size_t)n_q * 4, hipMemcpyHostToDevice));
    HIP_TRY(c, hipMemcpy(c->q_nrows.p, &n_q, 4, hipMemcpyHostToDevice));
    if (d_table) {
        c->attempts.release();
        c->attempts_ptr = dst; c->att_external = true; c->att_cap = n_q;
    } else {
        std::swap(c->attempts.p, own.p); std::swap(c->attempts.n, own.n);
        c->attempts_ptr = c->attempts.p; c->att_external = false; c->att_cap = cap;
    }
    return GROOT_OK;
}

int groot_hip_attempts_import(groot_ctx *c, const uint32_t *q_values, const uint32_t *counts, uint32_t n_rows)
{
    if (!c || (n_rows && (!q_values || !counts))) return GROOT_E_INVALID;
    if (!idle(c)) return fail(c, GROOT_E_STATE, "a batch is in flight");
    if (c->att_external) return fail(c, GROOT_E_STATE, "the table lives in a caller-owned buffer");
    std::vector<uint32_t> qs;
    if (int rc = table_rows(c, qs)) return rc;
    std::vector<uint32_t> all(qs);
    all.insert(all.end(), q_values, q_values + n_rows);
// ... 197 lines not shown
```

groot_amd/csrc/hip/kernels_lean.hpp:

```cpp
#pragma once

#include "kernels_common.hpp"

namespace groot {


#ifndef GROOT_LEAN_WAVES
#define GROOT_LEAN_WAVES 5
#endif
constexpr int kLeanWaves = GROOT_LEAN_WAVES;
#ifndef GROOT_LEAN_MAX_ITER
#define GROOT_LEAN_MAX_ITER 96
#endif
constexpr uint32_t kLeanMaxIter = GROOT_LEAN_MAX_ITER;

__device__ __forceinline__ uint64_t lean_lowmask(int n) { return n <= 0 ? 0ull : (n >= 32 ? ~0ull : ((1ull << (2 * n)) - 1ull)); }
__device__ __forceinline__ uint32_t lean_revcomp16(uint32_t v)
{
    uint32_t r = __brev(v);
    r = ((r & 0xAAAAAAAAu) >> 1) | ((r & 0x55555555u) << 1);
    return r ^ 0xAAAAAAAAu;
}
__device__ __forceinline__ uint64_t lean_funnel(uint32_t x0, uint32_t x1, uint32_t x2, uint32_t sh)
{
    return (uint64_t)__funnelshift_r(x0, x1, sh) | ((uint64_t)__funnelshift_r(x1, x2, sh) << 32);
}
__device__ __forceinline__ uint64_t lean_bits64(const uint32_t *wp, uint32_t bit)
{
    const uint32_t *q = wp + (bit >> 5);
    return lean_funnel(q[0], q[1], q[2], bit & 31u);
}

template <int PW, int NCH>
__global__ __launch_bounds__(kBlock, kLeanWaves) void align_lean_kernel(LeanArgs a)
{
    static_assert(PW == 3, "LeanNode holds three path words");
    static_assert(NCH >= 1 && NCH <= 8, "LeanExt holds bases [32, 256)");
    extern __shared__ __attribute__((aligned(16))) uint32_t lean_lds[];
    __shared__ unsigned long long red[4];
    uint32_t *my = lean_lds + (size_t)threadIdx.x * a.lds_stride_dw;
    uint32_t *W = my + (a.lds_stride_dw - 11u);
    enum : int { W_SEED, W_OFF0, W_L1HI, W_CNB, W_CNE, W_S0, W_SLEN, W_WIN };
#ifndef GROOT_LEAN_PRIO
#define GROOT_LEAN_PRIO -1
#endif
#if GROOT_LEAN_PRIO >= 0
    __builtin_amdgcn_s_setprio(GROOT_LEAN_PRIO);
#endif
    const uint32_t slot = blockIdx.x * kBlock + threadIdx.x;
    const uint32_t n_todo = min(a.n_reads, (uint32_t)__builtin_amdgcn_readfirstlane((int)a.ctr->seeded_reads));
    const bool stale = (a.ctr->flags & (kFlagSeedOverflow | kFlagQOverflow)) != 0;
#if defined(GROOT_WORK_COUNTERS) && GROOT_WORK_COUNTERS == 4
    const unsigned long long lw_t0 = wall_clock64();
#endif
    enum : uint32_t { ST_ADV, ST_GEN, ST_WALK, ST_SEED, ST_DONE, ST_DEFER, ST_IDLE };
    uint32_t st = ST_IDLE;
#if defined(GROOT_WORK_COUNTERS) && GROOT_WORK_COUNTERS == 4
    uint32_t why = 0;
#define LEAN_WHY(x) (why = (x))
#else
#define LEAN_WHY(x) ((void)0)
#endif
    uint32_t r = 0, len = 0, cnt = 0, vbits = 0;
    uint32_t g = kEmpty;
    if (slot < n_todo && !stale) {
        r = a.perm[slot];
        uint4 pk0 = make_uint4(0, 0, 0, 0), pk1 = pk0, pk2 = pk0, pk3 = pk0;
        if (a.packed) {
            const uint4 *pk = a.packed + (size_t)r * a.packed_q;
            pk0 = pk[0]; pk1 = pk[1];
            if (a.packed_q > 2u) { pk2 = pk[2]; pk3 = pk[3]; }
        }
        uint4 ra, rb;
        load32(a.read_rec + r, ra, rb);
        const uint32_t sc = ra.w;
        len = ra.z & ~kRecPacked;
        cnt = sc & (kRecSplit - 1u);
        vbits = (sc >> 24) & 0x3Fu;
        st = ST_ADV;
        if (cnt == 0u || cnt > 4u || (sc & kRecSplit) || (sc >> 31) || len > a.max_len || len < 12u) { st = ST_DEFER; LEAN_WHY(cnt > 4u ? 1 : 3); }
        else {
            uint32_t s0 = rb.x, s1 = cnt > 1u ? rb.y : kEmpty, s2 = cnt > 2u ? rb.z : kEmpty, s3 = cnt > 3u ? rb.w : kEmpty;
            { uint32_t t; if (s0 > s1) { t = s0; s0 = s1; s1 = t; } if (s2 > s3) { t = s2; s2 = s3; s3 = t; } if (s0 > s2) { t = s0; s0 = s2; s2 = t; }
              if (s1 > s3) { t = s1; s1 = s3; s3 = t; } if (s1 > s2) { t = s1; s1 = s2; s2 = t; } }
            const uint8_t *p = a.seq + ((uint64_t)ra.x | ((uint64_t)ra.y << 32));
            uint4 wa, wb;
            load32(a.win_rec + s0, wa, wb);
            const uint32_t ok = (uint32_t)a.win_ok[s0] & a.win_ok[cnt > 1u ? s1 : s0] & a.win_ok[cnt > 2u ? s2 : s0] & a.win_ok[cnt > 3u ? s3 : s0];
            my[0] = 0; my[1] = 0;
            uint32_t bad = 0;
            const uint32_t nd = (len + 15u) >> 4;
            if ((ra.z & kRecPacked) && a.packed) {
                const uint32_t c[16] = {pk0.x, pk0.y, pk0.z, pk0.w, pk1.x, pk1.y, pk1.z, pk1.w, pk2.x, pk2.y, pk2.z, pk2.w, pk3.x, pk3.y, pk3.z, pk3.w};
#pragma unroll
                for (int i = 0; i < 16; i++)
                    if ((uint32_t)i < nd) my[2 + i] = c[i];
            } else
            for (uint32_t i = 0; i < nd; i++) {
                uint4 v;
                __builtin_memcpy(&v, p + 16u * i, 16);
                const uint32_t x[4] = {v.x, v.y, v.z, v.w};
                uint32_t codes = 0;
#pragma unroll
                for (int j = 0; j < 4; j++) {
                    const uint32_t c = (x[j] >> 1) & 0x03030303u;
                    uint32_t diff = __builtin_amdgcn_perm(0u, 0x47544341u, c) ^ x[j];
                    const int left = (int)len - (int)(16u * i + 4u * j);
                    if (left < 4) diff = left <= 0 ? 0u : diff & ((1u << (8 * left)) - 1u);
                    bad |= diff;
                    uint32_t t = c | (c >> 6);
                    t = (t | (t >> 12)) & 0xFFu;
                    codes |= t << (8 * j);
                }
                my[2 + i] = codes;
            }
            my[2 + nd] = 0; my[3 + nd] = 0;
            g = wa.x;
            W[W_SEED] = wa.y; W[W_OFF0] = wa.z; W[W_L1HI] = wa.w;
            W[W_CNB] = wb.x; W[W_CNE] = wb.y; W[W_S0] = wb.z; W[W_SLEN] = wb.w;
            W[W_WIN] = s0; W[W_WIN + 1] = s1; W[W_WIN + 2] = s2; W[W_WIN + 3] = s3;
            if (bad || !ok) { st = ST_DEFER; LEAN_WHY(bad ? 4 : 5); }
        }
    }

    uint32_t si = 1;
    uint32_t done_graph = kEmpty, n_graphs = 1, ord = 0, calls = 1;
    uint32_t alns = 0;
    uint32_t rc = 0, level = 0, eff = len;
    uint32_t sbit = 64;
    auto chunk = [&](uint32_t d) -> uint64_t { return lean_bits64(my, sbit + 2u * d); };
    auto flip = [&]() {
        const uint32_t nd = (len + 15u) >> 4;
        for (uint32_t k2 = 0; 2u * k2 < nd; k2++) {
            const uint32_t x = my[2 + k2], y = my[1 + nd - k2];
            my[2 + k2] = lean_revcomp16(y);
            my[1 + nd - k2] = lean_revcomp16(x);
        }
        rc ^= 1u;
    };
    uint32_t p16 = 0;
    uint64_t need = 0;
    uint32_t pos = 0, sub = 0, lim = 0;
    uint32_t node0 = 0, noff0 = 0, cur = 0, cur_s0 = 0, coff = 0, dist = 0;
    bool cur_long = false;
    uint64_t cur64 = 0, m0 = 0, m1 = 0, m2 = 0;
    uint32_t emitted = 0, sp = 0;
    uint4 *stk = a.stk + (size_t)slot * 4;

    auto verdict = [&](uint32_t bit) -> bool { return si == 1u && (((vbits >> (rc ? 3 : 0)) >> bit) & 1u); };
    auto enter = [&](uint32_t lv) {
        const uint32_t off0 = W[W_OFF0], seed_len = W[W_SLEN];
        bool view = false;
        for (;;) {
            if (lv == 1u) {
                level = 1; view = true;
                if (!verdict(0)) {
                    pos = off0; lim = W[W_L1HI];
                    if (pos < lim) break;
                    lv = 2; continue;
                }
                lv = 3; continue;
            }
            if (lv == 2u) {
                level = 2; pos = W[W_CNB]; lim = W[W_CNE]; sub = 0;
                if (pos < lim) break;
                lv = 3; continue;
            }
            if (lv == 3u) {
                if (off0 >= seed_len) { lv = 5; continue; }
                if (verdict(1)) { lv = 4; continue; }
                level = 3; view = true; pos = 0; lim = 1;
                break;
            }
            if (lv == 4u) {
                if (verdict(2)) { lv = 5; continue; }
                level = 4; view = true; pos = 0; lim = 1;
                break;
            }
            if (rc == 0) { flip(); lv = 1; continue; }
            st = ST_SEED;
            return;
        }
        st = ST_GEN;
        if (view) {
            sbit = 64u + (rc ? 2u * (16u * ((len + 15u) >> 4) - len) : 0u) + (level == 3u ? 2u : 0u);
            eff = len - (level >= 3u ? 1u : 0u);
            p16 = (uint32_t)chunk(0) & 0xFFFFu;
            need = l2_bloom_bits(p16);
        }
    };
#if defined(GROOT_WORK_COUNTERS) && GROOT_WORK_COUNTERS == 4
    unsigned long long lw[12] = {0, 0, 0, 0, 0, 0, 0, 0, 0, 0, 0, 0};
    const unsigned long long lw_t1 = wall_clock64();
#define LEAN_EV(i, pred) do { const unsigned long long b__ = __ballot(pred); if (b__) { lw[i]++; lw[(i) + 4] += (unsigned long long)__popcll(b__); } } while (0)
#else
#define LEAN_EV(i, pred) ((void)0)
#endif
#ifdef GROOT_LEAN_PROBE
    if (GROOT_LEAN_PROBE == 1 && st <= ST_SEED) st = ST_DEFER;
#endif

    uint32_t iters = 0;
    while (__ballot(st <= ST_SEED)) {
        if (st <= ST_SEED && ++iters > kLeanMaxIter) { st = ST_DEFER; LEAN_WHY(10); }
        if (st == ST_SEED) {
            if (si >= cnt) st = ST_DONE;
            else {
                const uint32_t w = W[W_WIN + si];
                uint4 wa, wb;
                load32(a.win_rec + w, wa, wb);
                si++;
                if (wa.x != g) { g = wa.x; n_graphs++; }
                if (g != done_graph) {
                    calls |= 1u << (si - 1u);
                    W[W_SEED] = wa.y; W[W_OFF0] = wa.z; W[W_L1HI] = wa.w;
                    W[W_CNB] = wb.x; W[W_CNE] = wb.y; W[W_S0] = wb.z; W[W_SLEN] = wb.w;
                    if (rc) flip();
                    level = 0; emitted = 0;
                    st = ST_ADV;
                }
            }
        }
        if (st == ST_ADV) enter(level + 1u);
#if defined(GROOT_WORK_COUNTERS) && GROOT_WORK_COUNTERS == 4
        lw[8]++;
        LEAN_EV(0, st == ST_GEN && level == 1u); LEAN_EV(1, st == ST_GEN && level == 2u); LEAN_EV(2, st == ST_GEN && level >= 3u); LEAN_EV(3, st == ST_WALK);
#endif
        if (st == ST_GEN) {
            bool have = false;
            uint32_t c_node = 0, c_off = 0, c_s0 = 0, c_len = 0;
            if (level == 2u) {
                const uint4 e = a.cn_pre2[pos];
                const uint64_t G = (uint64_t)e.x | ((uint64_t)(e.y & 0xFFFFu) << 32);
                const uint32_t nlen = e.y >> 16, n = min(nlen, 11u);
                uint32_t j = sub;
                for (; j < n; j++) {
                    const uint32_t m = min(min(nlen - j, eff), 8u);
                    if ((((uint32_t)(G >> (2u * j)) ^ p16) & ((1u << (2u * m)) - 1u)) == 0u) break;
                }
                if (j < n) { have = true; c_node = e.z; c_off = j; c_s0 = e.w; c_len = nlen; sub = j + 1u; }
                else sub = n;
                if (sub >= n) { pos++; sub = 0; }
            } else {
                const uint32_t s0 = W[W_S0], slen = W[W_SLEN];
                const uint32_t from = level == 1u ? pos : W[W_OFF0];
                const uint64_t G = lean_bits64(a.bases2, 2u * (s0 + from));
                const uint32_t n = level == 1u ? min(24u, lim - pos) : 1u;
                uint32_t j = 0;
                for (; j < n; j++) {
                    const uint32_t m = min(min(slen - (from + j), eff), 8u);
                    if ((((uint32_t)(G >> (2u * j)) ^ p16) & ((1u << (2u * m)) - 1u)) == 0u) break;
                }
                if (j < n) { have = true; c_node = W[W_SEED]; c_off = from + j; c_s0 = s0; c_len = slen; }
                pos = level == 1u ? (j < n ? c_off + 1u : pos + n) : 1u;
            }
            if (have) {
                node0 = c_node; noff0 = c_off; cur = c_node; cur_s0 = c_s0; coff = c_off; dist = 0;
                cur_long = c_len > 32u;
                cur64 = chunk(0);
                m0 = m1 = m2 = ~0ull;
                st = ST_WALK;
            } else if (pos >= lim) st = ST_ADV;
        }
        if (st == ST_WALK) {
            const uint4 *q = reinterpret_cast<const uint4 *>(a.nodes + cur);
#if defined(GROOT_LEAN_PROBE) && GROOT_LEAN_PROBE == 2
            const uint4 q0 = q[0], q1 = q[1], q2 = q[2], q3 = make_uint4(~0u, ~0u, ~0u, ~0u);
#else
            const uint4 q0 = q[0], q1 = q[1], q2 = q[2], q3 = q[3];
#endif
            uint64_t gch[NCH];
#pragma unroll
            for (int c = 0; c < NCH; c++) gch[c] = 0;
            uint64_t l2b = ~0ull;
            if (dist == 0u && coff <= 10u && a.node_l2b) l2b = a.node_l2b[(size_t)cur * 11 + coff];
            if (coff != 0u) {
                const uint32_t bit = 2u * (cur_s0 + coff);
                const uint32_t *bp = a.bases2 + (bit >> 5);
                uint32_t x[2 * NCH + 1];
#pragma unroll
                for (int c = 0; c < 2 * NCH + 1; c++) x[c] = bp[c];
#pragma unroll
                for (int c = 0; c < NCH; c++) gch[c] = lean_funnel(x[2 * c], x[2 * c + 1], x[2 * c + 2], bit & 31u);
            } else if (cur_long) {
                const uint64_t *ep = a.ext[cur].b;
#pragma unroll
                for (int c = 1; c < NCH; c++) gch[c] = ep[c - 1];
            }
            const uint32_t seq_len = q0.y, dk = q0.z;
            if (coff == 0u) gch[0] = (uint64_t)q2.x | ((uint64_t)q2.y << 32);
            bool over = (l2b & need) != need;
            if (dk & kLeanNo) { st = ST_DEFER; LEAN_WHY(6); }
            else if (!over) {
                const uint32_t take = min(seq_len - coff, eff - dist);
                uint64_t diff = (gch[0] ^ cur64) & lean_lowmask((int)take);
                if (__ballot(take > 32u)) {
#pragma unroll
                    for (int c = 1; c < NCH; c++)
                        if (take > 32u * c) diff |= (gch[c] ^ chunk(dist + 32u * c)) & lean_lowmask((int)take - 32 * c);
                }
                over = diff != 0ull;
                if (!over) {
                    dist += take;
                    m0 &= (uint64_t)q2.z | ((uint64_t)q2.w << 32);
                    m1 &= (uint64_t)q3.x | ((uint64_t)q3.y << 32);
                    m2 &= (uint64_t)q3.z | ((uint64_t)q3.w << 32);
                    const bool any = (m0 | m1 | m2) != 0ull;
                    const uint32_t deg = dk & 7u;
                    if (dist == eff || deg == 0u) {
                        if (any) {
                            groot_trav t;
                            t.read_id = a.first_read_id + r; t.graph_id = g; t.node = node0; t.offset = noff0;
                            t.ord = (uint16_t)ord;
                            t.flags = (uint8_t)((rc ? GROOT_TRAV_RC : 0u) | (level == 3u ? GROOT_TRAV_START_CLIP : level == 4u ? GROOT_TRAV_END_CLIP : 0u) | (emitted == 0u ? GROOT_TRAV_FIRST : 0u));
                            t.reserved = 0;
                            if (ord == 0u) {
                                a.trav_first[r] = t;
                                a.mask_first[(size_t)r * PW] = m0; a.mask_first[(size_t)r * PW + 1] = m1; a.mask_first[(size_t)r * PW + 2] = m2;
                            } else {
                                const uint32_t shard = blockIdx.x & (kOvfShards - 1);
                                const uint32_t at = atomicAdd(&a.ovf_cnt[shard], 1u);
                                if (at < a.ovf_cap) {
                                    const size_t o = (size_t)shard * a.ovf_cap + at;
                                    a.ovf_trav[o] = t;
                                    a.ovf_mask[o * PW] = m0; a.ovf_mask[o * PW + 1] = m1; a.ovf_mask[o * PW + 2] = m2;
                                } else atomicOr(&a.ctr->flags, kFlagOvfOverflow);
                            }
                            ord++; emitted++;
                            alns += (uint32_t)(__popcll(m0) + __popcll(m1) + __popcll(m2));
                        }
                        over = true;
                    } else if (!any) over = true;
                    else {
                        cur64 = chunk(dist);
                        const uint32_t nextb = (uint32_t)cur64 & 3u;
                        const uint32_t ed[4] = {q1.x, q1.y, q1.z, q1.w};
                        uint32_t hits = 0, pick = 0, alt = 0;
                        bool wild = false;
#pragma unroll
                        for (int e = 0; e < 4; e++) {
                            const uint32_t code = (dk >> (8 + 4 * e)) & 15u;
                            if ((uint32_t)e < deg) {
                                wild |= code == 4u;
                                if (code == nextb) {
                                    const uint32_t nx = ed[e] | (((dk >> (24 + e)) & 1u) << 31);
                                    if (hits == 0u) pick = nx; else alt = nx;
                                    hits++;
                                }
                            }
                        }
                        if (wild || hits > 2u || (hits == 2u && sp == 2u)) { st = ST_DEFER; LEAN_WHY(wild ? 7 : hits > 2u ? 8 : 9); }
                        else if (hits == 0u) over = true;
                        else {
                            if (hits == 2u) {
                                stk[2 * sp] = make_uint4(alt, dist, (uint32_t)m0, (uint32_t)(m0 >> 32));
                                stk[2 * sp + 1] = make_uint4((uint32_t)m1, (uint32_t)(m1 >> 32), (uint32_t)m2, (uint32_t)(m2 >> 32));
                                sp++;
                            }
                            cur = pick & 0x7FFFFFFFu; coff = 0; cur_long = pick >> 31;
                        }
                    }
                }
            }
            if (over && st == ST_WALK) {
                if (sp) {
                    sp--;
                    const uint4 h0 = stk[2 * sp], h1 = stk[2 * sp + 1];
                    cur = h0.x & 0x7FFFFFFFu; cur_long = h0.x >> 31; coff = 0; dist = h0.y;
                    m0 = (uint64_t)h0.z | ((uint64_t)h0.w << 32);
                    m1 = (uint64_t)h1.x | ((uint64_t)h1.y << 32);
                    m2 = (uint64_t)h1.z | ((uint64_t)h1.w << 32);
                    cur64 = chunk(dist);
                } else if (emitted) { done_graph = g; st = ST_SEED; }
                else st = pos >= lim ? ST_ADV : ST_GEN;
            }
        }
    }

#if defined(GROOT_WORK_COUNTERS) && GROOT_WORK_COUNTERS == 4
    if ((threadIdx.x & 63) == 0) {
        const unsigned long long t2 = wall_clock64();
        for (int i = 0; i < 9; i++) atomicAdd(&a.ctr->dbg[140 + i], lw[i]);
        atomicAdd(&a.ctr->dbg[149], lw_t1 - lw_t0);
        atomicAdd(&a.ctr->dbg[150], t2 - lw_t1);
        atomicAdd(&a.ctr->dbg[151], 1ull);
    }
    for (uint32_t y = 1; y <= 10; y++) {
        const unsigned long long b = __ballot(st == ST_DEFER && why == y);
        if (b && (threadIdx.x & 63) == 0) atomicAdd(&a.ctr->dbg[160 + y], (unsigned long long)__popcll(b));
    }
    { const unsigned long long b = __ballot(st == ST_DONE && !ord); if (b && (threadIdx.x & 63) == 0) atomicAdd(&a.ctr->dbg[160], (unsigned long long)__popcll(b)); }
#endif
    const bool fin = st == ST_DONE;
    if (slot < n_todo) a.defer[slot] = st == ST_DEFER ? 1 : 0;
    unsigned long long n_alns = 0, mapped = 0, multimapped = 0;
    if (fin) {
        a.trav_cnt[r] = ord;
        mapped = 1;
        multimapped = n_graphs > 1u ? 1 : 0;
        n_alns = alns;
    }
    if (a.update_weights) {
        const uint32_t qrow = fin ? a.q_row[len - a.k + 1u] : 0u;
        const uint64_t cell = (uint64_t)qrow * a.n_windows + (fin ? W[W_WIN] : 0u);
        const unsigned long long here = __ballot(fin);
        const unsigned lane_ = threadIdx.x & 63u;
        const unsigned long long below = here & ((1ull << lane_) - 1ull);
        const int prev = below ? 63 - __builtin_clzll(below) : -1;
        const uint32_t plo = __shfl((uint32_t)cell, prev < 0 ? (int)lane_ : prev), phi = __shfl((uint32_t)(cell >> 32), prev < 0 ? (int)lane_ : prev);
        const bool head = fin && (prev < 0 || plo != (uint32_t)cell || phi != (uint32_t)(cell >> 32));
        const unsigned long long heads = __ballot(head);
        if (head) {
            const unsigned long long after = lane_ == 63u ? 0ull : heads & ~((2ull << lane_) - 1ull);
            const unsigned long long run = here & ~((1ull << lane_) - 1ull) & (after ? ((1ull << (__ffsll(after) - 1)) - 1ull) : ~0ull);
            atomicAdd(&a.attempts[cell], (uint32_t)__popcll(run));
        }
        if (fin && (calls >> 1))
            for (uint32_t i = 1; i < cnt; i++)
                if ((calls >> i) & 1u) atomicAdd(&a.attempts[(uint64_t)qrow * a.n_windows + W[W_WIN + i]], 1u);
    }
    n_alns = block_sum(n_alns, red);
    mapped = block_sum(mapped, red);
    multimapped = block_sum(multimapped, red);
    if (threadIdx.x == 0) {
        if (n_alns) atomicAdd(&a.ctr->alignments, n_alns);
        if (a.update_weights && mapped) atomicAdd(&a.ctr->mapped, mapped);
        if (a.update_weights && multimapped) atomicAdd(&a.ctr->multimapped, multimapped);
        if (mapped) atomicAdd(&a.ctr->lean_reads, (unsigned int)mapped);
    }
}

}
```

groot_amd/csrc/hip/launch.hpp:

```cpp
#pragma once

#include "device_types.hpp"

namespace groot {

bool seed_supported(uint32_t s, uint32_t max_k);
void launch_seed(uint32_t s, uint32_t max_k, const SeedArgs &a, bool dump, dim3 grid, size_t lds, hipStream_t st);

bool sig_supported(uint32_t s, uint32_t max_k, uint32_t k);
void launch_sig(uint32_t s, const SeedArgs &a, uint32_t max_len, hipStream_t st);
void launch_list(uint32_t s, const SeedArgs &a, dim3 list_grid, hipStream_t st);
void launch_text_lookup(uint32_t key_dwords, const SeedArgs &a, dim3 grid, size_t lds, hipStream_t st);

void launch_align(uint32_t pw, const AlignArgs &a, dim3 grid, hipStream_t st);
void launch_align_lean(uint32_t pw, const LeanArgs &a, dim3 grid, hipStream_t st);

}
```

groot_amd/device.py:

```python
import ctypes as C
import os

import numpy as np

from . import _ffi, host
from ._ffi import IndexView
from .host import GrootError

TRAV_DTYPE = np.dtype([("read_id", "<u4"), ("graph_id", "<u4"), ("node", "<u4"), ("offset", "<u4"), ("ord", "<u2"),
                       ("flags", "u1"), ("reserved", "u1")])
ALN_DTYPE = np.dtype([("read_id", "<u4"), ("graph_id", "<u4"), ("path_id", "<u4"), ("ref_id", "<u4"), ("pos", "<u4"),
                      ("start_clip", "u1"), ("end_clip", "u1"), ("rc", "u1"), ("secondary", "u1")])
SEED_DTYPE = np.dtype([("read_id", "<u4"), ("window_id", "<u4")])
TRAV_RC, TRAV_START_CLIP, TRAV_END_CLIP, TRAV_FIRST = 1, 2, 4, 8


class Params(C.Structure):
    _fields_ = [("containment_threshold", C.c_double), ("no_exact_align", C.c_uint32), ("max_read_len", C.c_uint32),
                ("max_batch_reads", C.c_uint32), ("max_seeds_per_read", C.c_uint32), ("max_batch_bases", C.c_uint64),
                ("keep_sketches", C.c_uint32), ("pipeline_depth", C.c_uint32), ("results_on_device", C.c_uint32),
                ("memo_budget_mb", C.c_uint32)]


MEMO_OFF = 0xFFFFFFFF
# ... 162 lines not shown
                 "packed": _ffi._np_view(b.packed, b.packed_cap, np.uint8), "seq_len": _ffi._np_view(b.seq_len, b.reads_cap, np.uint16),
                 "exc_pos": _ffi._np_view(b.exc_pos, b.exc_cap, np.uint64), "exc_byte": _ffi._np_view(b.exc_byte, b.exc_cap, np.uint8)}
        return views

    def submit_acquired(self, ticket, n_reads, n_exc=0, first_read_id=0):
        self._check(lib().groot_hip_submit_acquired(self._h, C.c_uint64(ticket), C.c_uint32(n_reads), C.c_uint64(n_exc), C.c_uint32(first_read_id)))

    def collect(self, check=True, copy=True):
        r = BatchResult()
        rc = lib().groot_hip_collect(self._h, C.byref(r))
        if rc < 0 and (check or not r.ticket):
            self._check(rc)
        n = int(r.n_travs)
        if r.travs and n:
            t = _ffi._np_view(C.cast(r.travs, C.POINTER(C.c_uint8)), n * TRAV_DTYPE.itemsize, np.uint8).view(TRAV_DTYPE)
            if copy:
                m = np.zeros((n, r.path_words), dtype=np.uint64)
                host._check(host.lib().groot_host_unpack_masks(C.byref(self.index.view), C.c_void_p(r.travs), C.c_uint64(n), C.c_void_p(r.masks),
                                                               _ffi.as_ptr(m, C.c_uint64)))
                t = t.copy()
            else:
                m = _ffi._np_view(C.cast(r.masks, C.POINTER(C.c_uint8)), int(r.n_mask_bytes), np.uint8)
        else:
            t, m = np.zeros(0, dtype=TRAV_DTYPE), np.zeros((0, self.path_words), dtype=np.uint64)
        return {"ticket": int(r.ticket), "first_read_id": int(r.first_read_id), "n_reads": int(r.n_reads), "counts": r.counts.as_dict(),
                "status": int(r.status), "n_travs": n, "travs": t, "masks": m, "n_mask_bytes": int(r.n_mask_bytes), "d_travs": r.d_travs,
                "d_masks": r.d_masks,
                "ms": {k: float(getattr(r.ms, k)) for k, _ in StageMs._fields_}}

    def release(self, ticket):
        self._check(lib().groot_hip_release(self._h, C.c_uint64(ticket)))

    def in_flight(self):
        a, b = C.c_uint32(), C.c_uint32()
        self._check(lib().groot_hip_in_flight(self._h, C.byref(a), C.byref(b)))
        return a.value, b.value

    def submit_device(self, d_seq_ptr, d_off_ptr, n_reads, first_read_id=0, max_len=0, mixed=False):
        if mixed:
            max_len |= 0x80000000
        self._check(lib().groot_hip_submit_device(self._h, C.c_void_p(d_seq_ptr), C.c_void_p(d_off_ptr), C.c_uint32(n_reads),
                                                  C.c_uint32(first_read_id), C.c_uint32(max_len)))

    def wait(self, check=True):
        c = Counts()
        rc = lib().groot_hip_wait(self._h, C.byref(c))
        self.last_rc = rc
        if check:
            self._check(rc)
        return c.as_dict()

    def seeds(self):
        n = C.c_uint64(0)
        self._check(lib().groot_hip_read_seeds(self._h, None, C.c_uint64(0), C.byref(n)))
        out = np.zeros(n.value, dtype=SEED_DTYPE)
        self._check(lib().groot_hip_read_seeds(self._h, out.ctypes.data_as(C.c_void_p), C.c_uint64(len(out)), C.byref(n)))
        return out

    def travs(self):
        n = C.c_uint64(0)
        self._check(lib().groot_hip_read_travs(self._h, None, None, C.c_uint64(0), C.byref(n)))
        t = np.zeros(n.value, dtype=TRAV_DTYPE)
        m = np.zeros((n.value, self.path_words), dtype=np.uint64)
        self._check(lib().groot_hip_read_travs(self._h, t.ctypes.data_as(C.c_void_p), _ffi.as_ptr(m, C.c_uint64),
                                               C.c_uint64(len(t)), C.byref(n)))
        return t, m

    def alns(self):
        t, m = self.travs()
        return expand_alns(self.index, t, m)

    def sketches(self):
        n = C.c_uint64(0)
        self._check(lib().groot_hip_read_sketches(self._h, None, C.c_uint64(0), C.byref(n)))
        out = np.zeros((n.value, self.s), dtype=np.uint64)
        self._check(lib().groot_hip_read_sketches(self._h, _ffi.as_ptr(out, C.c_uint64), C.c_uint64(n.value), C.byref(n)))
        return out

    def stage_ms(self):
        m = StageMs()
        self._check(lib().groot_hip_stage_ms(self._h, C.byref(m)))
        return {n: float(getattr(m, n)) for n, _ in StageMs._fields_}

    def attempts_shape(self):
        nq, nw = C.c_uint32(), C.c_uint32()
        self._check(lib().groot_hip_attempts_shape(self._h, C.byref(nq), C.byref(nw)))
        return nq.value, nw.value

    def attempts_device(self):
        p, nr, nw = C.c_void_p(), C.c_uint32(), C.c_uint32()
        self._check(lib().groot_hip_attempts_device(self._h, C.byref(p), C.byref(nr), C.byref(nw)))
        return p.value, nr.value, nw.value

    def attempts(self):
        nq, nw = self.attempts_shape()
        out = np.zeros((nq, nw), dtype=np.uint32)
        self._check(lib().groot_hip_attempts_read(self._h, _ffi.as_ptr(out, C.c_uint32), C.c_uint64(out.size)))
        return out

    def attempts_rows(self):
        nr, nw = C.c_uint32(), C.c_uint32()
        self._check(lib().groot_hip_attempts_export(self._h, None, None, C.c_uint32(0), C.byref(nr), C.byref(nw)))
        q = np.zeros(nr.value, dtype=np.uint32)
        cnt = np.zeros((nr.value, nw.value), dtype=np.uint32)
        self._check(lib().groot_hip_attempts_export(self._h, _ffi.as_ptr(q, C.c_uint32), _ffi.as_ptr(cnt, C.c_uint32), C.c_uint32(nr.value),
                                                    C.byref(nr), C.byref(nw)))
        return q, cnt

    def attempts_import(self, q_values, counts):
        q = np.ascontiguousarray(q_values, dtype=np.uint32)
        cnt = np.ascontiguousarray(counts, dtype=np.uint32)
        self._check(lib().groot_hip_attempts_import(self._h, _ffi.as_ptr(q, C.c_uint32), _ffi.as_ptr(cnt, C.c_uint32), C.c_uint32(len(q))))

    def attempts_layout(self, q_values, d_table=None):
        q = np.ascontiguousarray(q_values, dtype=np.uint32)
        self._check(lib().groot_hip_attempts_layout(self._h, _ffi.as_ptr(q, C.c_uint32), C.c_uint32(len(q)), C.c_void_p(d_table or 0)))

    def attempts_reset(self):
        self._check(lib().groot_hip_attempts_reset(self._h))

    def sketch(self, seq_concat, seq_off):
        seq = np.ascontiguousarray(seq_concat, dtype=np.uint8)
        off = np.ascontiguousarray(seq_off, dtype=np.uint64)
        out = np.zeros((len(off) - 1, self.s), dtype=np.uint64)
        self._check(lib().groot_hip_sketch(self._h, _ffi.as_ptr(seq, C.c_uint8), _ffi.as_ptr(off, C.c_uint64),
                                           C.c_uint32(len(off) - 1), _ffi.as_ptr(out, C.c_uint64)))
        return out


def attempts_allreduce(aligners):
    arr = (C.c_void_p * len(aligners))(*[a._h for a in aligners])
    rc = lib().groot_hip_attempts_allreduce(arr, C.c_int(len(aligners)))
    aligners[0]._check(rc)


def weights_rows(index, q_values, counts):
    q = np.ascontiguousarray(q_values, dtype=np.uint32)
    cnt = np.ascontiguousarray(counts, dtype=np.uint32)
    v = index.view
    kf = np.zeros(v.n_nodes, dtype=np.float64)
    kt = np.zeros(v.n_graphs, dtype=np.uint64)
    host._check(host.lib().groot_host_weights_rows(C.byref(v), _ffi.as_ptr(q, C.c_uint32), C.c_uint32(len(q)), _ffi.as_ptr(cnt, C.c_uint32),
                                                   _ffi.as_ptr(kf, C.c_double), _ffi.as_ptr(kt, C.c_uint64)))
    return kf, kt


def weights(index, attempts):
    att = np.ascontiguousarray(attempts, dtype=np.uint32)
    v = index.view
    kf = np.zeros(v.n_nodes, dtype=np.float64)
    kt = np.zeros(v.n_graphs, dtype=np.uint64)
    host._check(host.lib().groot_host_weights(C.byref(v), _ffi.as_ptr(att, C.c_uint32), C.c_uint32(att.shape[0]),
                                              _ffi.as_ptr(kf, C.c_double), _ffi.as_ptr(kt, C.c_uint64)))
    return kf, kt


def prune(index, kmer_freq, min_cov=1.0):
    v = index.view
    gk = np.zeros(v.n_graphs, dtype=np.uint8)
    pk = np.zeros(v.n_paths, dtype=np.uint8)
    nr = np.zeros(v.n_nodes, dtype=np.uint8)
    kf = np.ascontiguousarray(kmer_freq, dtype=np.float64)
    host._check(host.lib().groot_host_prune(C.byref(v), _ffi.as_ptr(kf, C.c_double), C.c_double(min_cov), _ffi.as_ptr(gk, C.c_uint8),
                                            _ffi.as_ptr(pk, C.c_uint8), _ffi.as_ptr(nr, C.c_uint8)))
    return gk, pk, nr
```

include/groot_hip.h:

```cpp
#ifndef GROOT_HIP_H
#define GROOT_HIP_H

#include <stddef.h>
#include <stdint.h>

#include "groot_host.h"
#include "groot_index.h"

#ifdef __cplusplus
extern "C" {
#endif

typedef struct groot_ctx groot_ctx;

typedef struct groot_params {
    double   containment_threshold;
    uint32_t no_exact_align;
    uint32_t max_read_len;
    uint32_t max_batch_reads;
    uint32_t max_seeds_per_read;
    uint64_t max_batch_bases;
    uint32_t keep_sketches;
    uint32_t pipeline_depth;
    uint32_t results_on_device;
// ... 25 lines not shown
} groot_counts;

typedef struct groot_stage_ms {
    float h2d, sketch_seed, align, sort, total, schedule, d2h, unpack;
    float first_seed_kernel, order_kernel;
    float list_pass, wall;
    float lean_pass;
} groot_stage_ms;

int groot_hip_device_count(int *n);
const char *groot_hip_last_error(const groot_ctx *ctx);

int groot_hip_open(groot_ctx **out, int device_id, const groot_index_view *idx, const groot_params *p);
#define GROOT_OPEN_BACKGROUND 1u
int groot_hip_open_flags(groot_ctx **out, int device_id, const groot_index_view *idx, const groot_params *p, uint32_t flags);
int groot_hip_open_wait(groot_ctx *ctx);
int groot_hip_open_abandon(groot_ctx *ctx);
void groot_hip_close(groot_ctx *ctx);

typedef struct groot_open_stats {
    double open_ms;
    double memo_ms;
    uint64_t memo_strings;
    uint64_t memo_tabulated;
    uint64_t memo_entries;
    uint64_t text_entries;
    uint64_t memo_hbm_bytes;
} groot_open_stats;
int groot_hip_open_stats(const groot_ctx *ctx, groot_open_stats *out);

int groot_hip_set_stream(groot_ctx *ctx, void *hip_stream);
int groot_hip_stream_join(groot_ctx *ctx, void *hip_stream);
int groot_hip_redo_status(groot_ctx *ctx, const uint32_t **d_status, uint32_t *redo_mask);
int groot_hip_set_profiling(groot_ctx *ctx, int enable);


int groot_hip_submit(groot_ctx *ctx, const uint8_t *seq_concat, const uint64_t *seq_off, uint32_t n_reads,
                     uint32_t first_read_id);
int groot_hip_submit_packed(groot_ctx *ctx, const uint8_t *packed, const uint64_t *seq_off, uint32_t n_reads,
                            uint32_t first_read_id, const uint64_t *exc_pos, const uint8_t *exc_byte, uint64_t n_exc);
int groot_hip_submit_packed16(groot_ctx *ctx, const uint8_t *packed, const uint16_t *seq_len, uint32_t n_reads,
                              uint32_t first_read_id, const uint64_t *exc_pos, const uint8_t *exc_byte, uint64_t n_exc);
typedef struct groot_batch_buffers {
    uint64_t ticket;
    uint8_t *packed;
    uint16_t *seq_len;
    uint64_t *exc_pos;
    uint8_t *exc_byte;
    uint64_t packed_cap, exc_cap;
    uint32_t reads_cap, reserved;
} groot_batch_buffers;
int groot_hip_acquire(groot_ctx *ctx, groot_batch_buffers *out);
int groot_hip_submit_acquired(groot_ctx *ctx, uint64_t ticket, uint32_t n_reads, uint64_t n_exc, uint32_t first_read_id);
#define GROOT_MAXLEN_MIXED 0x80000000u
int groot_hip_submit_device(groot_ctx *ctx, const void *d_seq, const void *d_seq_off, uint32_t n_reads,
                            uint32_t first_read_id, uint32_t max_len);

typedef struct groot_batch_result {
    uint64_t ticket;
    uint32_t first_read_id, n_reads;
    groot_counts counts;
    const groot_trav *travs;
    const uint8_t *masks;
    const uint32_t *mask_ckpt;
    uint64_t n_mask_bytes;
    uint64_t n_travs;
    const void *d_travs;
    const void *d_masks;
    uint32_t path_words;
    int32_t status;
    groot_stage_ms ms;
} groot_batch_result;
int groot_hip_collect(groot_ctx *ctx, groot_batch_result *out);
int groot_hip_release(groot_ctx *ctx, uint64_t ticket);
int groot_hip_in_flight(groot_ctx *ctx, uint32_t *submitted_not_collected, uint32_t *free_slots);

int groot_hip_wait(groot_ctx *ctx, groot_counts *counts);
int groot_hip_read_travs(groot_ctx *ctx, groot_trav *out, uint64_t *masks , uint64_t cap,
                         uint64_t *n);
int groot_hip_read_seeds(groot_ctx *ctx, groot_seed *out, uint64_t cap, uint64_t *n);
int groot_hip_read_sketches(groot_ctx *ctx, uint64_t *out , uint64_t cap_reads,
                            uint64_t *n_reads);
int groot_hip_stage_ms(groot_ctx *ctx, groot_stage_ms *out);

int groot_hip_attempts_export(groot_ctx *ctx, uint32_t *q_values, uint32_t *counts, uint32_t cap_rows, uint32_t *n_rows,
                              uint32_t *n_windows);
int groot_hip_attempts_layout(groot_ctx *ctx, const uint32_t *q_values, uint32_t n_q, void *d_table);
int groot_hip_attempts_import(groot_ctx *ctx, const uint32_t *q_values, const uint32_t *counts, uint32_t n_rows);
int groot_hip_attempts_device(groot_ctx *ctx, void **d_table, uint32_t *n_rows, uint32_t *n_windows);
int groot_hip_attempts_reset(groot_ctx *ctx);
int groot_hip_attempts_allreduce(groot_ctx *const *ctxs, int n_ctx);
int groot_hip_attempts_shape(groot_ctx *ctx, uint32_t *n_q, uint32_t *n_windows);
int groot_hip_attempts_read(groot_ctx *ctx, uint32_t *out, uint64_t n_elems);

int groot_hip_sketch(groot_ctx *ctx, const uint8_t *seq_concat, const uint64_t *seq_off, uint32_t n, uint64_t *out);

#ifdef __cplusplus
}
#endif
#endif
```

Baseline: 2005.

## Add path-text first-pass alignment kernel with sparse-table mask intersection

Adds a new first-pass alignment kernel that is on by default. It matches reads against linearised path texts, checking 32 bases per 64-bit word with XOR, instead of walking the graph node by node. Path membership over a run of nodes is taken from a precomputed sparse table of ANDed node masks, so a whole range costs two lookups. Extra traversal records go to a small hold buffer and then the overflow list, and reads that cannot be handled this way go back to the old lean/full kernels. The cost is host-side table building and more device memory, plus more branch divergence and more register pressure in the kernel.

```diff
diff --git a/groot_amd/csrc/hip/align.hip b/groot_amd/csrc/hip/align.hip
--- a/groot_amd/csrc/hip/align.hip
+++ b/groot_amd/csrc/hip/align.hip
@@ -27,4 +27,13 @@
     else hipLaunchKernelGGL((align_lean_kernel<3, 8>), grid, dim3(kBlock), lds, st, a);
 }
 
+void launch_align_path(uint32_t pw, const LeanArgs &a, dim3 grid, hipStream_t st)
+{
+    if (pw != 3) return;
+    const size_t lds = (size_t)kBlock * a.lds_stride_dw * 4;
+    if (a.max_len <= 128) hipLaunchKernelGGL((align_path_kernel<3, 4>), grid, dim3(kBlock), lds, st, a);
+    else if (a.max_len <= 160) hipLaunchKernelGGL((align_path_kernel<3, 5>), grid, dim3(kBlock), lds, st, a);
+    else hipLaunchKernelGGL((align_path_kernel<3, 8>), grid, dim3(kBlock), lds, st, a);
 }
+
+}
diff --git a/groot_amd/csrc/hip/device_types.hpp b/groot_amd/csrc/hip/device_types.hpp
--- a/groot_amd/csrc/hip/device_types.hpp
+++ b/groot_amd/csrc/hip/device_types.hpp
@@ -37,6 +37,7 @@
     unsigned int seeded_reads;
     unsigned int tab_reads;
     unsigned int lean_reads;
+    unsigned int path_reads;
     unsigned long long dbg[192];
 };
 
@@ -273,6 +274,12 @@
     uint32_t *ovf_cnt;
     uint32_t ovf_cap;
     DeviceCounters *ctr;
+    const uint4 *path_node;
+    const uint32_t *path_text;
+    const uint32_t *path_tag;
+    const uint32_t *path_nodes;
+    const uint64_t *path_tab;
+    uint4 *hold;
 };
 
 __host__ __device__ inline uint32_t lean_stride_dw(uint32_t max_len) { return (((max_len + 15u) >> 4) + 15u) | 1u; }
diff --git a/groot_amd/csrc/hip/groot_hip.hip b/groot_amd/csrc/hip/groot_hip.hip
--- a/groot_amd/csrc/hip/groot_hip.hip
+++ b/groot_amd/csrc/hip/groot_hip.hip
@@ -21,6 +21,7 @@
 #include "../common/cpus.hpp"
 #include "../common/view_check.hpp"
 #include "kernels_misc.hpp"
+#include "kernels_path.hpp"
 #include "launch.hpp"
 
 using namespace groot;
@@ -64,7 +65,7 @@
 };
 
 struct Knobs {
-    bool no_outcome_table = false, no_text_table = false, no_sig = false, force_rccl = false, small_buffers = false, open_stats = false, poison = false, lean = false;
+    bool no_outcome_table = false, no_text_table = false, no_sig = false, force_rccl = false, small_buffers = false, open_stats = false, poison = false, lean = false, no_path = false;
     static Knobs read()
     {
         Knobs k;
@@ -73,6 +74,7 @@
         k.small_buffers = getenv("GROOT_TEST_SMALL_BUFFERS") != nullptr;  k.open_stats = getenv("GROOT_OPEN_STATS") != nullptr;
         k.poison = getenv("GROOT_TEST_POISON") != nullptr;
         k.lean = getenv("GROOT_LEAN") != nullptr;
+        k.no_path = getenv("GROOT_NO_PATH_PASS") != nullptr;
         return k;
     }
 };
@@ -89,6 +91,9 @@
     bool sig_used = false;
     uint32_t packed_q = 0;
     bool lean_used = false;
+    bool path_used = false;
+    uint32_t path_reads = 0;
+    float path_ms = 0;
     bool one_len = false;
     uint64_t n_bases = 0, n_exc = 0;
     enum Input { IN_ASCII, IN_PACKED, IN_PACKED16, IN_DEVICE } input = IN_ASCII;
@@ -176,6 +181,10 @@
     DevBuf<uint8_t> win_ok;
     DevBuf<uint4> lean_stk;
     bool lean = false;
+    bool path = false;
+    DevBuf<uint4> path_node, path_hold;
+    DevBuf<uint32_t> path_text, path_tag, path_nodes;
+    DevBuf<uint64_t> path_tab;
     DevBuf<WinRec> win_rec;
     DevBuf<ExactEntry> exact;
     DevBuf<SigEntry> sig;
@@ -337,6 +346,103 @@
     for (uint32_t c : {3u, 11u})
         if (pw <= c) return c;
     return 0;
+}
+
+struct PathTables {
+    std::vector<uint4> node;
+    std::vector<uint32_t> text, tag;
+    std::vector<uint32_t> nodes;
+    std::vector<uint64_t> tab;
+    uint32_t n_text_paths = 0;
+    size_t n_bases = 0;
+};
+static bool build_path_tables(const groot_index_view *v, PathTables &pt)
+{
+    auto code_of = [](uint8_t b) -> int { return b == 'A' ? 0 : b == 'C' ? 1 : b == 'T' ? 2 : b == 'G' ? 3 : -1; };
+    auto nlen = [&](uint32_t n) { return v->node_seq_off[n + 1] - v->node_seq_off[n]; };
+    std::vector<uint32_t> gnode(v->n_nodes, 0);
+    for (uint32_t g = 0; g < v->n_graphs; g++)
+        for (uint32_t n = v->graph_node_off[g]; n < v->graph_node_off[g + 1]; n++) gnode[n] = g;
+    std::vector<uint8_t> flag(v->n_nodes, 0);
+    for (uint32_t n = 0; n < v->n_nodes; n++) {
+        const uint32_t e0 = v->node_edge_off[n], deg = v->node_edge_off[n + 1] - e0;
+        uint32_t seen = 0;
+        bool f = deg > 4;
+        for (uint32_t e = 0; e < deg && !f; e++) {
+            const uint32_t ch = v->edges[e0 + e];
+            if (nlen(ch) == 0) continue;
+            const int cd = code_of(v->bases[v->node_seq_off[ch]]);
+            if (cd < 0 || (seen >> cd) & 1u) f = true;
+            else seen |= 1u << cd;
+        }
+        flag[n] = f;
+    }
+    auto has_edge = [&](uint32_t a, uint32_t b) {
+        for (uint32_t e = v->node_edge_off[a]; e < v->node_edge_off[a + 1]; e++)
+            if (v->edges[e] == b) return true;
+        return false;
+    };
+    std::vector<std::vector<std::pair<uint32_t, uint32_t>>> pl(v->n_paths);
+    for (uint32_t n = 0; n < v->n_nodes; n++)
+        for (uint32_t i = v->node_np_off[n]; i < v->node_np_off[n + 1]; i++) {
+            const uint32_t gp = v->graph_path_off[gnode[n]] + v->np_path[i];
+            if (gp < v->n_paths) pl[gp].push_back({v->np_pos[i], n});
+        }
+    std::vector<uint8_t> ok(v->n_paths, 0);
+    size_t total = 0;
+    for (uint32_t p = 0; p < v->n_paths; p++) {
+        auto &L = pl[p];
+        std::sort(L.begin(), L.end());
+        bool good = !L.empty();
+        for (size_t i = 0; good && i < L.size(); i++) {
+            if (nlen(L[i].second) == 0) good = false;
+            else if (i + 1 < L.size() && ((uint64_t)L[i].first + nlen(L[i].second) != L[i + 1].first || !has_edge(L[i].second, L[i + 1].second))) good = false;
+        }
+        if (!good) continue;
+        ok[p] = 1;
+        pt.n_text_paths++;
+        total += (uint64_t)L.back().first + nlen(L.back().second) - L.front().first;
+    }
+    pt.n_bases = total;
+    if (total + 512 >= (1ull << 31)) return false;
+    pt.text.assign(total / 16 + 20, 0);
+    pt.tag.assign(total / 16 + 20, 0);
+    pt.node.assign((size_t)v->n_nodes * 2, make_uint4(kEmpty, 0, 0, 0));
+    const uint32_t pw = std::min<uint32_t>(v->path_words, 3);
+    size_t at = 0;
+    for (uint32_t p = 0; p < v->n_paths; p++) {
+        if (!ok[p]) continue;
+        const auto &L = pl[p];
+        const uint32_t n = (uint32_t)L.size(), nbase = (uint32_t)pt.nodes.size(), tbase = (uint32_t)(pt.tab.size() / 3);
+        const uint32_t tend = (uint32_t)(at + (L.back().first + nlen(L.back().second) - L.front().first));
+        uint32_t levels = 1;
+        while ((2ull << (levels - 1)) <= n) levels++;
+        pt.tab.resize(pt.tab.size() + (size_t)3 * levels * n, 0);
+        uint64_t *T = pt.tab.data() + (size_t)3 * tbase;
+        for (uint32_t i = 0; i < n; i++)
+            for (uint32_t w = 0; w < pw; w++) T[(size_t)3 * i + w] = v->node_mask[(size_t)L[i].second * v->path_words + w];
+        for (uint32_t k = 1; k < levels; k++)
+            for (uint32_t i = 0; i + (1u << k) <= n; i++)
+                for (uint32_t w = 0; w < 3; w++)
+                    T[(size_t)3 * ((size_t)k * n + i) + w] = T[(size_t)3 * ((size_t)(k - 1) * n + i) + w] & T[(size_t)3 * ((size_t)(k - 1) * n + i + (1u << (k - 1))) + w];
+        for (uint32_t i = 0; i < n; i++) {
+            const uint32_t nd = L[i].second, s0 = v->node_seq_off[nd], len = nlen(nd);
+            if (pt.node[2 * (size_t)nd].x == kEmpty) {
+                pt.node[2 * (size_t)nd] = make_uint4((uint32_t)at, i, tend, nbase);
+                pt.node[2 * (size_t)nd + 1] = make_uint4(tbase, n, 0, 0);
+            }
+            pt.nodes.push_back(nd);
+            for (uint32_t j = 0; j < len; j++, at++) {
+                const int cd = code_of(v->bases[s0 + j]);
+                const uint32_t tg = j == 0 ? 1u | ((i > 0 && flag[L[i - 1].second]) ? 2u : 0u) : (cd < 0 ? 2u : 0u);
+                pt.text[at >> 4] |= (uint32_t)(cd < 0 ? 0 : cd) << (2 * (at & 15));
+                pt.tag[at >> 4] |= tg << (2 * (at & 15));
+            }
+        }
+    }
+    if (pt.nodes.empty()) pt.nodes.push_back(0);
+    if (pt.tab.empty()) pt.tab.assign(3, 0);
+    return true;
 }
 
 template <int PW> void build_node_records(const groot_index_view *v, std::vector<unsigned char> &out)
@@ -518,7 +624,7 @@
         const uint32_t stride_dw = ((s->max_len + 3) / 4 + 1) | 1u;
         a.list_stride_dw = list_lds_stride(stride_dw);
         HIP_TRY(c, hipMemsetAsync(c->todo_count.p, 0, sizeof(uint32_t), c->stream));
-        if (c->lean && !c->tab_capture && w->packed.p) { a.packed = w->packed.p; a.packed_q = s->max_len <= 128 ? 2u : 4u; }
+        if ((c->lean || c->path) && !c->tab_capture && w->packed.p) { a.packed = w->packed.p; a.packed_q = s->max_len <= 128 ? 2u : 4u; }
         s->packed_q = a.packed ? a.packed_q : 0;
         launch_sig(c->s, a, s->max_len, c->stream);
         HIP_TRY(c, hipGetLastError());
@@ -613,7 +719,9 @@
     uint32_t blocks = std::min<uint32_t>((s->n_reads + kBlock - 1) / kBlock, c->align_threads / kBlock);
     if (c->dfs_frac < kSparseBelow && c->dfs_frac * (double)s->n_reads < 16.0 * (double)(blocks * (kBlock / 64))) blocks = std::max(1u, blocks / 2);
     else if (c->dfs_frac >= kSparseBelow && c->dfs_frac < 0.6 && !s->mixed_len && blocks >= 4) blocks /= 2;
-    if (c->lean && !c->tab_capture && c->lean_left_frac < 0.25) {
+    s->lean_used = c->lean && !c->tab_capture && s->n_reads && s->max_len <= kLeanMaxLen && c->dfs_frac >= 0.02;
+    s->path_used = c->path && !c->tab_capture && s->n_reads && s->max_len <= kLeanMaxLen && c->dfs_frac >= 0.02;
+    if ((s->lean_used || s->path_used) && c->lean_left_frac < 0.25) {
         uint32_t want = (uint32_t)(c->lean_left_frac * 1.25 * (double)s->n_reads / 64.0 / (kBlock / 64)) + 1u;
         blocks = std::max(1u, std::min(blocks, std::max(want, c->n_cu)));
     }
@@ -641,8 +749,7 @@
     a.ctr = s->d_ctr.p;
     HIP_TRY(c, hipMemsetAsync(c->ovf_cnt.p, 0, (kOvfShards + 2) * sizeof(uint32_t), c->astream));
     const uint32_t lean_stride = lean_stride_dw(s->max_len);
-    s->lean_used = c->lean && !c->tab_capture && s->n_reads && s->max_len <= kLeanMaxLen && c->dfs_frac >= 0.02;
-    if (s->lean_used) {
+    if (s->lean_used || s->path_used) {
         LeanArgs l{};
         l.nodes = c->lean_nodes.p; l.ext = c->lean_ext.p; l.bases2 = c->bases2.p; l.cn_pre2 = c->cn_pre2.p; l.win_ok = c->win_ok.p;
         l.win_rec = c->dix.win_rec; l.node_l2b = c->dix.node_l2b; l.q_row = c->q_row.p;
@@ -655,7 +762,11 @@
         l.defer = w->defer.p; l.ctr = s->d_ctr.p;
         l.stk = c->lean_stk.p; l.ovf_trav = c->ovf_trav.p; l.ovf_mask = c->ovf_mask.p; l.ovf_cnt = c->ovf_cnt.p; l.ovf_cap = c->ovf_cap;
         const uint32_t lean_blocks = std::min<uint32_t>((s->n_reads + kBlock - 1) / kBlock, (uint32_t)(c->dfs_frac * 1.05 * (double)s->n_reads / kBlock) + 64u);
-        launch_align_lean(c->pw, l, dim3(lean_blocks), c->astream);
+        if (s->path_used) {
+            l.path_node = c->path_node.p; l.path_text = c->path_text.p; l.path_tag = c->path_tag.p; l.path_nodes = c->path_nodes.p; l.path_tab = c->path_tab.p;
+            l.hold = c->path_hold.p;
+            launch_align_path(c->pw, l, dim3(lean_blocks), c->astream);
+        } else launch_align_lean(c->pw, l, dim3(lean_blocks), c->astream);
         HIP_TRY(c, hipGetLastError());
         size_t tb = 0;
         rocprim::counting_iterator<uint32_t> ids(0u);
@@ -1002,7 +1113,7 @@
             merged.flags = keep | again.flags;
             merged.q_rows = again.q_rows;
             merged.mask_words = again.mask_words;
-            merged.todo_reads = again.todo_reads; merged.tab_reads = again.tab_reads; merged.lean_reads = again.lean_reads;
+            merged.todo_reads = again.todo_reads; merged.tab_reads = again.tab_reads; merged.lean_reads = again.lean_reads; merged.path_reads = again.path_reads;
             h = merged;
         } else h = again;
     }
@@ -1014,6 +1125,7 @@
     o.full_sketch_reads = (s->sig_used || s->text_used) ? h.todo_reads : s->n_reads;
     o.walked_reads = h.seeded_reads;
     o.lean_reads = h.lean_reads;
+    s->path_reads = s->path_used ? h.path_reads : 0;
     if (s->status == GROOT_OK) {
         char buf[256];
         if (h.flags & kFlagLongRead) { s->status = GROOT_E_NOSPACE; snprintf(buf, sizeof buf, "a read is longer than max_read_len=%u", c->prm.max_read_len); s->status_msg = buf; }
@@ -1053,6 +1165,9 @@
                 (double)h.dbg[144] / nw, (double)h.dbg[145] / nw, (double)h.dbg[146] / nw, (double)h.dbg[147] / nw, (double)h.dbg[149] / nw / 100.0, (double)h.dbg[150] / nw / 100.0);
         fprintf(stderr, "[groot lean] finished without an alignment %llu; left to align_kernel: seeds > 4: %llu, byte > T / length: %llu, byte other than ACGT: %llu, window with an N: %llu, node with an N: %llu, N ahead: %llu, three neighbours: %llu, third pending: %llu, too many steps: %llu\n",
                 h.dbg[160], h.dbg[161], h.dbg[163], h.dbg[164], h.dbg[165], h.dbg[166], h.dbg[167], h.dbg[168], h.dbg[169], h.dbg[170]);
+        if (s->path_used)
+            fprintf(stderr, "[groot path] left to align_kernel: node on no path with a text %llu, event on the start base %llu, more than %u records %llu; segments ended: empty path set %llu, read's end %llu, end of the path's text %llu, flagged boundary %llu, jump %llu\n",
+                    h.dbg[171], h.dbg[172], kPathHold + 1, h.dbg[173], h.dbg[176], h.dbg[177], h.dbg[178], h.dbg[179], h.dbg[180]);
     }
 #elif defined(GROOT_WORK_COUNTERS)
     for (int e = 0; e < 32; e++)
@@ -1077,7 +1192,10 @@
 #endif
     if (s->n_reads) c->trav_per_read = (double)s->n_trav / (double)s->n_reads;
     if (s->n_reads && !c->tab_capture) c->dfs_frac = (double)h.seeded_reads / (double)s->n_reads;
-    if (s->n_reads && !c->tab_capture && s->lean_used) c->lean_left_frac = (double)(h.seeded_reads - std::min(h.seeded_reads, h.lean_reads)) / (double)s->n_reads;
+    if (s->n_reads && !c->tab_capture && (s->lean_used || s->path_used)) {
+        const uint32_t first = s->path_used ? h.path_reads : h.lean_reads;
+        c->lean_left_frac = (double)(h.seeded_reads - std::min(h.seeded_reads, first)) / (double)s->n_reads;
+    }
     if (s->n_reads && (s->sig_used || s->text_used)) c->todo_frac = (double)h.todo_reads / (double)s->n_reads;
     if (s->n_reads && !c->tab_capture && c->dix.text_tab) {
         c->text_hit_frac = s->text_used ? 1.0 - (double)h.todo_reads / (double)s->n_reads : (double)h.tab_reads / (double)s->n_reads;
@@ -1139,8 +1257,9 @@
         (void)hipEventElapsedTime(&s->ms.first_seed_kernel, s->ev[7], s->ev[8]);
         (void)hipEventElapsedTime(&s->ms.order_kernel, s->ev[9], s->ev[10]);
         (void)hipEventElapsedTime(&s->ms.list_pass, s->ev[8], s->ev[12]);
-        s->ms.lean_pass = 0;
+        s->ms.lean_pass = 0; s->path_ms = 0;
         if (s->lean_used) (void)hipEventElapsedTime(&s->ms.lean_pass, s->ev[11], s->ev[13]);
+        if (s->path_used) (void)hipEventElapsedTime(&s->path_ms, s->ev[11], s->ev[13]);
         (void)hipEventElapsedTime(&s->ms.wall, s->ev[1], s->ev[5]);
         if (!c->prm.results_on_device) (void)hipEventElapsedTime(&s->ms.d2h, s->ev_d2h0, s->ev_d2h);
     }
@@ -1915,7 +2034,21 @@
         HIP_TRY(c, upload(c->node_rec, recs.data(), recs.size()));
     }
     c->lean = c->pw == 3 && c->kn.lean && !c->prm.no_exact_align;
-    if (c->lean) {
+    c->path = c->pw == 3 && !c->kn.lean && !c->kn.no_path && !c->prm.no_exact_align;
+    PathTables pt;
+    if (c->path) c->path = build_path_tables(v, pt);
+    if (c->path) {
+        HIP_TRY(c, upload(c->path_node, pt.node.data(), pt.node.size()));
+        HIP_TRY(c, upload(c->path_text, pt.text.data(), pt.text.size()));
+        HIP_TRY(c, upload(c->path_tag, pt.tag.data(), pt.tag.size()));
+        HIP_TRY(c, upload(c->path_nodes, pt.nodes.data(), pt.nodes.size()));
+        HIP_TRY(c, upload(c->path_tab, pt.tab.data(), pt.tab.size()));
+        if (c->kn.open_stats)
+            fprintf(stderr, "[groot open] path tables: %u of %u paths with a text, %zu bases; node records %.2f MB, text + tags %.2f MB, node lists %.2f MB, sparse tables %.2f MB\n",
+                    pt.n_text_paths, v->n_paths, pt.n_bases, pt.node.size() * 16 / 1e6, (pt.text.size() + pt.tag.size()) * 4 / 1e6, pt.nodes.size() * 4 / 1e6, pt.tab.size() * 8 / 1e6);
+        pt = PathTables();
+    }
+    if (c->lean || c->path) {
         auto code_of = [](uint8_t b) -> int { return b == 'A' ? 0 : b == 'C' ? 1 : b == 'T' ? 2 : b == 'G' ? 3 : -1; };
         std::vector<uint32_t> b2((size_t)(v->n_bases + 15) / 16 + 20, 0);
         for (uint64_t i = 0; i < v->n_bases; i++) {
@@ -2247,7 +2380,7 @@
         HIP_TRY(c, w.read_rec.alloc(R));
         HIP_TRY(c, w.perm.alloc(R));
         HIP_TRY(c, w.perm_count.alloc(4));
-        if (c->lean) {
+        if (c->lean || c->path) {
             HIP_TRY(c, w.perm2.alloc(R));
             HIP_TRY(c, w.perm2_count.alloc(4));
             HIP_TRY(c, w.defer.alloc(R));
@@ -2263,7 +2396,8 @@
         HIP_TRY(c, hipMemset(w.vcount.p, 0, 4 * sizeof(uint32_t)));
     }
     HIP_TRY(c, c->trav_off.alloc(R));
-    if (c->lean) HIP_TRY(c, c->lean_stk.alloc((size_t)R * 4));
+    if (c->lean || c->path) HIP_TRY(c, c->lean_stk.alloc((size_t)R * 4));
+    if (c->path) HIP_TRY(c, c->path_hold.alloc((size_t)R * 3 * kPathHold));
     HIP_TRY(c, c->ovf_cnt.alloc(kOvfShards + 2));
     if (int rc = alloc_ovf(c, c->kn.small_buffers ? 2u : std::max<uint32_t>(256, R / kOvfShards / 4))) return rc;
     int n_cu = 256;
@@ -2786,6 +2920,16 @@
     return GROOT_OK;
 }
 
+int groot_hip_path_pass_stats(groot_ctx *c, uint32_t *ran, uint64_t *reads, float *ms)
+{
+    if (!c || !ran || !reads || !ms) return GROOT_E_INVALID;
+    const Slot *s = c->waited;
+    *ran = s && s->path_used ? 1u : 0u;
+    *reads = *ran ? s->path_reads : 0;
+    *ms = *ran ? s->path_ms : 0.0f;
+    return GROOT_OK;
+}
+
 static int table_rows(groot_ctx *c, std::vector<uint32_t> &q_of_row)
 {
     if (int rc = drain(c)) return rc;
diff --git a/groot_amd/csrc/hip/kernels_lean.hpp b/groot_amd/csrc/hip/kernels_lean.hpp
--- a/groot_amd/csrc/hip/kernels_lean.hpp
+++ b/groot_amd/csrc/hip/kernels_lean.hpp
@@ -1,6 +1,7 @@
 #pragma once
 
 #include "kernels_common.hpp"
+#include "kernels_path.hpp"
 
 namespace groot {
 
@@ -31,8 +32,8 @@
     return lean_funnel(q[0], q[1], q[2], bit & 31u);
 }
 
-template <int PW, int NCH>
-__global__ __launch_bounds__(kBlock, kLeanWaves) void align_lean_kernel(LeanArgs a)
+template <int PW, int NCH, bool PATH>
+__device__ __forceinline__ void first_pass_body(const LeanArgs &a)
 {
     static_assert(PW == 3, "LeanNode holds three path words");
     static_assert(NCH >= 1 && NCH <= 8, "LeanExt holds bases [32, 256)");
@@ -146,6 +147,36 @@
     uint64_t cur64 = 0, m0 = 0, m1 = 0, m2 = 0;
     uint32_t emitted = 0, sp = 0;
     uint4 *stk = a.stk + (size_t)slot * 4;
+    uint32_t t = 0, tend = 0, idx = 0, nbase = 0, tbase = 0, pnn = 0;
+    bool pn_need = false;
+    uint4 *hold = PATH ? a.hold + (size_t)slot * (3 * kPathHold) : nullptr;
+    auto emit = [&]() {
+        groot_trav t_;
+        t_.read_id = a.first_read_id + r; t_.graph_id = g; t_.node = node0; t_.offset = noff0;
+        t_.ord = (uint16_t)ord;
+        t_.flags = (uint8_t)((rc ? GROOT_TRAV_RC : 0u) | (level == 3u ? GROOT_TRAV_START_CLIP : level == 4u ? GROOT_TRAV_END_CLIP : 0u) | (emitted == 0u ? GROOT_TRAV_FIRST : 0u));
+        t_.reserved = 0;
+        if (ord == 0u) {
+            a.trav_first[r] = t_;
+            a.mask_first[(size_t)r * PW] = m0; a.mask_first[(size_t)r * PW + 1] = m1; a.mask_first[(size_t)r * PW + 2] = m2;
+        } else if (PATH) {
+            if (ord > kPathHold) { st = ST_DEFER; LEAN_WHY(13); return; }
+            uint4 *h = hold + 3u * (ord - 1u);
+            h[0] = make_uint4(g, node0, noff0, (uint32_t)t_.ord | ((uint32_t)t_.flags << 16));
+            h[1] = make_uint4((uint32_t)m0, (uint32_t)(m0 >> 32), (uint32_t)m1, (uint32_t)(m1 >> 32));
+            h[2] = make_uint4((uint32_t)m2, (uint32_t)(m2 >> 32), 0u, 0u);
+        } else {
+            const uint32_t shard = blockIdx.x & (kOvfShards - 1);
+            const uint32_t at = atomicAdd(&a.ovf_cnt[shard], 1u);
+            if (at < a.ovf_cap) {
+                const size_t o = (size_t)shard * a.ovf_cap + at;
+                a.ovf_trav[o] = t_;
+                a.ovf_mask[o * PW] = m0; a.ovf_mask[o * PW + 1] = m1; a.ovf_mask[o * PW + 2] = m2;
+            } else atomicOr(&a.ctr->flags, kFlagOvfOverflow);
+        }
+        ord++; emitted++;
+        alns += (uint32_t)(__popcll(m0) + __popcll(m1) + __popcll(m2));
+    };
 
     auto verdict = [&](uint32_t bit) -> bool { return si == 1u && (((vbits >> (rc ? 3 : 0)) >> bit) & 1u); };
     auto enter = [&](uint32_t lv) {
@@ -195,6 +226,12 @@
 #define LEAN_EV(i, pred) do { const unsigned long long b__ = __ballot(pred); if (b__) { lw[i]++; lw[(i) + 4] += (unsigned long long)__popcll(b__); } } while (0)
 #else
 #define LEAN_EV(i, pred) ((void)0)
+#endif
+#if defined(GROOT_WORK_COUNTERS) && GROOT_WORK_COUNTERS == 4
+    uint32_t stops[5] = {0, 0, 0, 0, 0};
+#define LEAN_STOP(i) (stops[i]++)
+#else
+#define LEAN_STOP(i) ((void)0)
 #endif
 #ifdef GROOT_LEAN_PROBE
     if (GROOT_LEAN_PROBE == 1 && st <= ST_SEED) st = ST_DEFER;
@@ -254,7 +291,12 @@
                 if (j < n) { have = true; c_node = W[W_SEED]; c_off = from + j; c_s0 = s0; c_len = slen; }
                 pos = level == 1u ? (j < n ? c_off + 1u : pos + n) : 1u;
             }
-            if (have) {
+            if (have && PATH) {
+                node0 = c_node; noff0 = c_off; cur = c_node; coff = c_off; dist = 0;
+                m0 = m1 = m2 = ~0ull;
+                pn_need = true;
+                st = ST_WALK;
+            } else if (have) {
                 node0 = c_node; noff0 = c_off; cur = c_node; cur_s0 = c_s0; coff = c_off; dist = 0;
                 cur_long = c_len > 32u;
                 cur64 = chunk(0);
@@ -262,7 +304,77 @@
                 st = ST_WALK;
             } else if (pos >= lim) st = ST_ADV;
         }
-        if (st == ST_WALK) {
+        if (PATH && st == ST_WALK) {
+            bool over = false;
+            if (pn_need) {
+                const uint4 *pq = a.path_node + 2u * cur;
+                const uint4 p0 = pq[0], p1 = pq[1];
+                if (p0.x == kEmpty) { st = ST_DEFER; LEAN_WHY(11); }
+                else { t = p0.x + coff; idx = p0.y; tend = p0.z; nbase = p0.w; tbase = p1.x; pnn = p1.y; pn_need = false; }
+            }
+            if (st == ST_WALK) {
+                const PathStop ps = path_segment<NCH>(a.path_text, a.path_tag, t, min(eff - dist, tend - t), [&](uint32_t d) { return chunk(dist + d); });
+                if (ps.e == 0u) { st = ST_DEFER; LEAN_WHY(12); }
+                else if (ps.e != kEmpty && !ps.at_start) over = true;
+                else {
+                    const uint32_t stop = ps.e == kEmpty ? ps.n : ps.e, last = idx + ps.ns;
+                    const bool step = ps.e != kEmpty || dist + ps.n < eff;
+                    uint32_t prev = 0, nextn = kEmpty;
+                    if (step) { prev = a.path_nodes[nbase + last]; if (last + 1u < pnn) nextn = a.path_nodes[nbase + last + 1u]; }
+                    uint64_t r0, r1, r2;
+                    path_range_and<PW>(a.path_tab, tbase, pnn, idx, last, r0, r1, r2);
+                    m0 &= r0; m1 &= r1; m2 &= r2;
+                    dist += stop;
+                    if ((m0 | m1 | m2) == 0ull) { over = true; LEAN_STOP(0); }
+                    else if (!step) { emit(); over = true; LEAN_STOP(1); }
+                    else {
+                        const uint4 *q = reinterpret_cast<const uint4 *>(a.nodes + prev);
+                        const uint4 q0 = q[0], q1 = q[1];
+                        const uint32_t dk = q0.z, deg = dk & 7u;
+                        LEAN_STOP(ps.e == kEmpty ? 2 : ps.flagged ? 3 : 4);
+                        if (deg == 0u) { emit(); over = true; }
+                        else if (deg > 4u) { st = ST_DEFER; LEAN_WHY(8); }
+                        else {
+                            const uint32_t nextb = (uint32_t)chunk(dist) & 3u;
+                            const uint32_t ed[4] = {q1.x, q1.y, q1.z, q1.w};
+                            uint32_t hits = 0, pick = 0, alt = 0;
+                            bool wild = false;
+#pragma unroll
+                            for (int e = 0; e < 4; e++) {
+                                const uint32_t code = (dk >> (8 + 4 * e)) & 15u;
+                                if ((uint32_t)e < deg) {
+                                    wild |= code == 4u;
+                                    if (code == nextb) { if (hits == 0u) pick = ed[e]; else alt = ed[e]; hits++; }
+                                }
+                            }
+                            if (wild || hits > 2u || (hits == 2u && sp == 2u)) { st = ST_DEFER; LEAN_WHY(wild ? 7 : hits > 2u ? 8 : 9); }
+                            else if (hits == 0u) over = true;
+                            else {
+                                if (hits == 2u) {
+                                    stk[2 * sp] = make_uint4(alt, dist, (uint32_t)m0, (uint32_t)(m0 >> 32));
+                                    stk[2 * sp + 1] = make_uint4((uint32_t)m1, (uint32_t)(m1 >> 32), (uint32_t)m2, (uint32_t)(m2 >> 32));
+                                    sp++;
+                                }
+                                if (pick == nextn) { t += stop; idx = last + 1u; }
+                                else { cur = pick; coff = 0; pn_need = true; }
+                            }
+                        }
+                    }
+                }
+            }
+            if (over && st == ST_WALK) {
+                if (sp) {
+                    sp--;
+                    const uint4 h0 = stk[2 * sp], h1 = stk[2 * sp + 1];
+                    cur = h0.x; coff = 0; dist = h0.y; pn_need = true;
+                    m0 = (uint64_t)h0.z | ((uint64_t)h0.w << 32);
+                    m1 = (uint64_t)h1.x | ((uint64_t)h1.y << 32);
+                    m2 = (uint64_t)h1.z | ((uint64_t)h1.w << 32);
+                } else if (emitted) { done_graph = g; st = ST_SEED; }
+                else st = pos >= lim ? ST_ADV : ST_GEN;
+            }
+        }
+        if (!PATH && st == ST_WALK) {
             const uint4 *q = reinterpret_cast<const uint4 *>(a.nodes + cur);
 #if defined(GROOT_LEAN_PROBE) && GROOT_LEAN_PROBE == 2
             const uint4 q0 = q[0], q1 = q[1], q2 = q[2], q3 = make_uint4(~0u, ~0u, ~0u, ~0u);
@@ -308,27 +420,7 @@
                     const bool any = (m0 | m1 | m2) != 0ull;
                     const uint32_t deg = dk & 7u;
                     if (dist == eff || deg == 0u) {
-                        if (any) {
-                            groot_trav t;
-                            t.read_id = a.first_read_id + r; t.graph_id = g; t.node = node0; t.offset = noff0;
-                            t.ord = (uint16_t)ord;
-                            t.flags = (uint8_t)((rc ? GROOT_TRAV_RC : 0u) | (level == 3u ? GROOT_TRAV_START_CLIP : level == 4u ? GROOT_TRAV_END_CLIP : 0u) | (emitted == 0u ? GROOT_TRAV_FIRST : 0u));
-                            t.reserved = 0;
-                            if (ord == 0u) {
-                                a.trav_first[r] = t;
-                                a.mask_first[(size_t)r * PW] = m0; a.mask_first[(size_t)r * PW + 1] = m1; a.mask_first[(size_t)r * PW + 2] = m2;
-                            } else {
-                                const uint32_t shard = blockIdx.x & (kOvfShards - 1);
-                                const uint32_t at = atomicAdd(&a.ovf_cnt[shard], 1u);
-                                if (at < a.ovf_cap) {
-                                    const size_t o = (size_t)shard * a.ovf_cap + at;
-                                    a.ovf_trav[o] = t;
-                                    a.ovf_mask[o * PW] = m0; a.ovf_mask[o * PW + 1] = m1; a.ovf_mask[o * PW + 2] = m2;
-                                } else atomicOr(&a.ctr->flags, kFlagOvfOverflow);
-                            }
-                            ord++; emitted++;
-                            alns += (uint32_t)(__popcll(m0) + __popcll(m1) + __popcll(m2));
-                        }
+                        if (any) emit();
                         over = true;
                     } else if (!any) over = true;
                     else {
@@ -390,12 +482,34 @@
         if (b && (threadIdx.x & 63) == 0) atomicAdd(&a.ctr->dbg[160 + y], (unsigned long long)__popcll(b));
     }
     { const unsigned long long b = __ballot(st == ST_DONE && !ord); if (b && (threadIdx.x & 63) == 0) atomicAdd(&a.ctr->dbg[160], (unsigned long long)__popcll(b)); }
+    for (uint32_t y = 11; y <= 13; y++) {
+        const unsigned long long b = __ballot(st == ST_DEFER && why == y);
+        if (b && (threadIdx.x & 63) == 0) atomicAdd(&a.ctr->dbg[160 + y], (unsigned long long)__popcll(b));
+    }
+    if (PATH)
+        for (int i = 0; i < 5; i++) if (stops[i]) atomicAdd(&a.ctr->dbg[176 + i], (unsigned long long)stops[i]);
 #endif
     const bool fin = st == ST_DONE;
     if (slot < n_todo) a.defer[slot] = st == ST_DEFER ? 1 : 0;
     unsigned long long n_alns = 0, mapped = 0, multimapped = 0;
     if (fin) {
         a.trav_cnt[r] = ord;
+        if (PATH)
+            for (uint32_t o = 1; o < ord; o++) {
+                const uint4 h0 = hold[3 * (o - 1)], h1 = hold[3 * (o - 1) + 1], h2 = hold[3 * (o - 1) + 2];
+                groot_trav t_;
+                t_.read_id = a.first_read_id + r; t_.graph_id = h0.x; t_.node = h0.y; t_.offset = h0.z;
+                t_.ord = (uint16_t)(h0.w & 0xFFFFu); t_.flags = (uint8_t)(h0.w >> 16); t_.reserved = 0;
+                const uint32_t shard = blockIdx.x & (kOvfShards - 1);
+                const uint32_t at = atomicAdd(&a.ovf_cnt[shard], 1u);
+                if (at < a.ovf_cap) {
+                    const size_t q = (size_t)shard * a.ovf_cap + at;
+                    a.ovf_trav[q] = t_;
+                    a.ovf_mask[q * PW] = (uint64_t)h1.x | ((uint64_t)h1.y << 32);
+                    a.ovf_mask[q * PW + 1] = (uint64_t)h1.z | ((uint64_t)h1.w << 32);
+                    a.ovf_mask[q * PW + 2] = (uint64_t)h2.x | ((uint64_t)h2.y << 32);
+                } else atomicOr(&a.ctr->flags, kFlagOvfOverflow);
+            }
         mapped = 1;
         multimapped = n_graphs > 1u ? 1 : 0;
         n_alns = alns;
@@ -426,8 +540,16 @@
         if (n_alns) atomicAdd(&a.ctr->alignments, n_alns);
         if (a.update_weights && mapped) atomicAdd(&a.ctr->mapped, mapped);
         if (a.update_weights && multimapped) atomicAdd(&a.ctr->multimapped, multimapped);
-        if (mapped) atomicAdd(&a.ctr->lean_reads, (unsigned int)mapped);
-    }
+        if (mapped) atomicAdd(PATH ? &a.ctr->path_reads : &a.ctr->lean_reads, (unsigned int)mapped);
+    }
+#undef LEAN_WHY
+#undef LEAN_EV
+#undef LEAN_STOP
 }
 
+template <int PW, int NCH>
+__global__ __launch_bounds__(kBlock, kLeanWaves) void align_lean_kernel(LeanArgs a) { first_pass_body<PW, NCH, false>(a); }
+template <int PW, int NCH>
+__global__ __launch_bounds__(kBlock, kPathWaves) void align_path_kernel(LeanArgs a) { first_pass_body<PW, NCH, true>(a); }
+
 }
diff --git a/groot_amd/csrc/hip/kernels_path.hpp b/groot_amd/csrc/hip/kernels_path.hpp
--- /dev/null
+++ b/groot_amd/csrc/hip/kernels_path.hpp
@@ -0,0 +1,63 @@
+#pragma once
+
+#include "kernels_common.hpp"
+
+namespace groot {
+
+
+#ifndef GROOT_PATH_WAVES
+#define GROOT_PATH_WAVES 4
+#endif
+constexpr int kPathWaves = GROOT_PATH_WAVES;
+constexpr uint32_t kPathHold = 4;
+
+struct PathStop {
+    uint32_t n;
+    uint32_t e;
+    uint32_t ns;
+    bool at_start, flagged;
+};
+
+__device__ __forceinline__ uint64_t path_funnel(uint32_t x0, uint32_t x1, uint32_t x2, uint32_t sh)
+{
+    return (uint64_t)__funnelshift_r(x0, x1, sh) | ((uint64_t)__funnelshift_r(x1, x2, sh) << 32);
+}
+template <int NCH, typename View>
+__device__ __forceinline__ PathStop path_segment(const uint32_t *text, const uint32_t *tag, uint32_t t, uint32_t n, View view)
+{
+    constexpr uint64_t k55 = 0x5555555555555555ull;
+    const uint32_t bit = 2u * t, sh = bit & 31u;
+    const uint32_t *cp = text + (bit >> 5), *tp = tag + (bit >> 5);
+    uint32_t x[2 * NCH + 1], y[2 * NCH + 1];
+#pragma unroll
+    for (int c = 0; c < 2 * NCH + 1; c++) { x[c] = cp[c]; y[c] = tp[c]; }
+    PathStop ps{n, kEmpty, 0u, false, false};
+#pragma unroll
+    for (int c = 0; c < NCH; c++) {
+        if (ps.e == kEmpty && n > 32u * c) {
+            const uint64_t lim = (n >= 32u * (c + 1) ? ~0ull : ((1ull << (2 * (n - 32u * c))) - 1ull)) & (c == 0 ? ~3ull : ~0ull);
+            const uint64_t g = path_funnel(x[2 * c], x[2 * c + 1], x[2 * c + 2], sh), tg = path_funnel(y[2 * c], y[2 * c + 1], y[2 * c + 2], sh);
+            const uint64_t d = g ^ view(32u * c), lo = tg & k55, hi = (tg >> 1) & k55;
+            const uint64_t mis = (d | (d >> 1)) & k55 & ~(hi & ~lo) & (n >= 32u * (c + 1) ? ~0ull : ((1ull << (2 * (n - 32u * c))) - 1ull));
+            const uint64_t ev = mis | (hi & lo & lim);
+            const uint64_t starts = lo & lim;
+            if (ev) {
+                const uint32_t j = (uint32_t)__builtin_ctzll(ev) >> 1;
+                ps.e = 32u * c + j;
+                ps.at_start = (lo >> (2 * j)) & 1u;
+                ps.flagged = (hi >> (2 * j)) & ps.at_start;
+                ps.ns += (uint32_t)__popcll(starts & ((1ull << (2 * j)) - 1ull));
+            } else ps.ns += (uint32_t)__popcll(starts);
+        }
+    }
+    return ps;
+}
+template <int PW>
+__device__ __forceinline__ void path_range_and(const uint64_t *ptab, uint32_t tbase, uint32_t n, uint32_t lo, uint32_t hi, uint64_t &r0, uint64_t &r1, uint64_t &r2)
+{
+    const uint32_t lv = 31u - __builtin_clz(hi - lo + 1u);
+    const uint64_t *pa = ptab + (size_t)PW * (tbase + (size_t)lv * n + lo), *pb = ptab + (size_t)PW * (tbase + (size_t)lv * n + hi + 1u - (1u << lv));
+    r0 = pa[0] & pb[0]; r1 = pa[1] & pb[1]; r2 = pa[2] & pb[2];
+}
+
+}
diff --git a/groot_amd/csrc/hip/launch.hpp b/groot_amd/csrc/hip/launch.hpp
--- a/groot_amd/csrc/hip/launch.hpp
+++ b/groot_amd/csrc/hip/launch.hpp
@@ -14,5 +14,6 @@
 
 void launch_align(uint32_t pw, const AlignArgs &a, dim3 grid, hipStream_t st);
 void launch_align_lean(uint32_t pw, const LeanArgs &a, dim3 grid, hipStream_t st);
+void launch_align_path(uint32_t pw, const LeanArgs &a, dim3 grid, hipStream_t st);
 
 }
diff --git a/groot_amd/device.py b/groot_amd/device.py
--- a/groot_amd/device.py
+++ b/groot_amd/device.py
@@ -268,6 +268,11 @@
         self._check(lib().groot_hip_stage_ms(self._h, C.byref(m)))
         return {n: float(getattr(m, n)) for n, _ in StageMs._fields_}
 
+    def path_pass_stats(self):
+        ran, reads, ms = C.c_uint32(), C.c_uint64(), C.c_float()
+        self._check(lib().groot_hip_path_pass_stats(self._h, C.byref(ran), C.byref(reads), C.byref(ms)))
+        return {"ran": bool(ran.value), "reads": int(reads.value), "ms": float(ms.value)}
+
     def attempts_shape(self):
         nq, nw = C.c_uint32(), C.c_uint32()
         self._check(lib().groot_hip_attempts_shape(self._h, C.byref(nq), C.byref(nw)))
diff --git a/include/groot_hip.h b/include/groot_hip.h
--- a/include/groot_hip.h
+++ b/include/groot_hip.h
@@ -131,6 +131,7 @@
 int groot_hip_read_sketches(groot_ctx *ctx, uint64_t *out , uint64_t cap_reads,
                             uint64_t *n_reads);
 int groot_hip_stage_ms(groot_ctx *ctx, groot_stage_ms *out);
+int groot_hip_path_pass_stats(groot_ctx *ctx, uint32_t *ran, uint64_t *reads, float *ms);
 
 int groot_hip_attempts_export(groot_ctx *ctx, uint32_t *q_values, uint32_t *counts, uint32_t cap_rows, uint32_t *n_rows,
                               uint32_t *n_windows);
```

After: 2154, median of 6. 7.4% higher.
